# lukashermann/hulc

Hardware: AMD Instinct MI355X
Metric: trajectory-windows/sec (seq_len=32, bs=64/GPU) (higher is better)
Workload: dtype bf16; 1 GPU; HULC training step, vision goal only (use_clip_auxiliary_loss=false), B=64 windows/GPU, seq_len=32, 200x200 static + 84x84 gripper fp32 NCHW frames, fwd+loss+bwd+Adam, dropout 0.1; global_batch=64, seq_len=32, parallelism=dp1

## Files before the change

### hulc_amd/csrc/capi.hip

```cpp
#include <cstdarg>
#include <cstdio>
#include <cstring>
#include <cstdlib>
#include <cmath>
#include <algorithm>
#include <stdexcept>

#include "engine.h"
#include "sbert.h"
#include "store_gather.h"
#include "store_stage.h"

using namespace hulc_bf16;

static thread_local char g_err[1024] = "";
void hulc_set_error(const char* fmt, ...) {
    va_list ap;
    va_start(ap, fmt);
    vsnprintf(g_err, sizeof(g_err), fmt, ap);
    va_end(ap);
}

struct hulc_ctx {
    IEngine* e = nullptr;
// ... 316 lines not shown
    HULC_K_16BIT("hulc_k_enc_tail_bwd", k_enc_tail_bwd(Nf, ldemb, a, b, demb, stream));
}
int hulc_k_tr_layer_fwd(int32_t dtype, const hulc_tr_layer_job* job, int32_t B, int32_t S, int32_t ln_in, float dp, void* stream) {
    HULC_K_16BIT("hulc_k_tr_layer_fwd", k_tr_layer_fwd(job, B, S, ln_in, dp, stream));
}
int hulc_k_tr_ffn_bwd(int32_t dtype, const hulc_tr_ffn_bwd_job* job, int32_t B, int32_t S, int32_t bcast, float bdiv, float dp, void* stream) {
    HULC_K_16BIT("hulc_k_tr_ffn_bwd", k_tr_ffn_bwd(job, B, S, bcast, bdiv, dp, stream));
}
int hulc_k_tr_attn_bwd(int32_t dtype, const hulc_tr_attn_bwd_job* job, int32_t B, int32_t S, int32_t nparts, int64_t part_stride, float dp, void* stream) {
    HULC_K_16BIT("hulc_k_tr_attn_bwd", k_tr_attn_bwd(job, B, S, nparts, (long long)part_stride, dp, stream));
}
int hulc_k_gemm_multi(int32_t dtype, int32_t form, const hulc_gemm_epi_job* jobs, int32_t n, int32_t sh, int32_t* ran, void* stream) {
    HULC_K_16BIT("hulc_k_gemm_multi", k_gemm_multi(form, jobs, n, sh, ran, stream));
}
#undef HULC_K_16BIT
int hulc_k_gemm_epi(int32_t dtype, const hulc_gemm_epi_job* job, int32_t kernel, int32_t* ran, void* stream) {
    if (dtype == HULC_DTYPE_F16) return hulc_f16::k_gemm_epi(1, job, kernel, ran, stream);
    if (dtype != HULC_DTYPE_F32 && dtype != HULC_DTYPE_BF16) { hulc_set_error("hulc_k_gemm_epi: unknown dtype %d", (int)dtype); return 1; }
    return hulc_bf16::k_gemm_epi(dtype == HULC_DTYPE_BF16 ? 1 : 0, job, kernel, ran, stream);
}
int hulc_k_gemm_pick(int32_t dtype, int32_t M, int32_t N, int32_t K, int64_t lda, int64_t ldb, int32_t* pick, int32_t* bk) {
    if (dtype != HULC_DTYPE_F32 && dtype != HULC_DTYPE_BF16 && dtype != HULC_DTYPE_F16) { hulc_set_error("hulc_k_gemm_pick: unknown dtype %d", (int)dtype); return 1; }
    return hulc_bf16::k_gemm_pick(dtype != HULC_DTYPE_F32, M, N, K, (long long)lda, (long long)ldb, pick, bk);
}
int hulc_k_gemm_wgrad_nsplit(int32_t dtype, int32_t M, int32_t N, int32_t K, int32_t* nsplit, int32_t* big) {
    if (dtype != HULC_DTYPE_F32 && dtype != HULC_DTYPE_BF16 && dtype != HULC_DTYPE_F16) { hulc_set_error("hulc_k_gemm_wgrad_nsplit: unknown dtype %d", (int)dtype); return 1; }
    return hulc_bf16::k_gemm_wgrad_nsplit(dtype != HULC_DTYPE_F32, M, N, K, nsplit, big);
}
int hulc_k_logistic_loss(int32_t dtype, int32_t wide, const float* heads, int32_t ldh, const float* actions, const float* robot_obs, int32_t B, int32_t S,
                         int32_t n_mix, int32_t n_dim, int32_t num_classes, float log_scale_min, float gripper_alpha, int32_t gripper_control,
                         int32_t discrete_gripper, float grad_scale, const float* lscale, float* row_loss, float* a_tcp_out, void* dheads, void* stream) {
    if (dtype == HULC_DTYPE_F16)
        return hulc_f16::k_logistic_loss(1, wide, heads, ldh, actions, robot_obs, B, S, n_mix, n_dim, num_classes, log_scale_min, gripper_alpha, gripper_control,
                                         discrete_gripper, grad_scale, lscale, row_loss, a_tcp_out, dheads, stream);
    if (dtype != HULC_DTYPE_F32 && dtype != HULC_DTYPE_BF16) { hulc_set_error("hulc_k_logistic_loss: unknown dtype %d", (int)dtype); return 1; }
    return hulc_bf16::k_logistic_loss(dtype == HULC_DTYPE_BF16, wide, heads, ldh, actions, robot_obs, B, S, n_mix, n_dim, num_classes, log_scale_min, gripper_alpha,
                                      gripper_control, discrete_gripper, grad_scale, lscale, row_loss, a_tcp_out, dheads, stream);
}
#define HULC_K_ANY(name, fn, ...)                                                                                                     \
    if (dtype == HULC_DTYPE_F16) return hulc_f16::fn(1, __VA_ARGS__);                                                                  \
    if (dtype != HULC_DTYPE_F32 && dtype != HULC_DTYPE_BF16) { hulc_set_error(name ": unknown dtype %d", (int)dtype); return 1; }      \
    return hulc_bf16::fn(dtype == HULC_DTYPE_BF16 ? 1 : 0, __VA_ARGS__)
int hulc_k_plan_kl_sample(const float* pr_logits, const float* pp_logits, int32_t B, int32_t NCAT, int32_t NCLS, const int32_t* idx_in, int32_t* idx_out, float* probs,
                          float* kl_cat, float* dpp, float* dpr, float w_pp, float w_pr, uint64_t seed, const float* lscale, void* stream) {
    return hulc_bf16::k_plan_kl_sample(pr_logits, pp_logits, B, NCAT, NCLS, idx_in, idx_out, probs, kl_cat, dpp, dpr, w_pp, w_pr, (unsigned long long)seed, lscale, stream);
}
int hulc_k_st_softmax_bwd(int32_t dtype, const float* probs, const float* dplan, const float* dpr_kl, const float* dpp_kl, int32_t rows, int32_t NCLS, float* out, void* out_t,
                          void* dpp_t, void* stream) {
    HULC_K_ANY("hulc_k_st_softmax_bwd", k_st_softmax_bwd, probs, dplan, dpr_kl, dpp_kl, rows, NCLS, out, out_t, dpp_t, stream);
}
int hulc_k_plan_gather(int32_t dtype, const void* w_t, const int32_t* idx, int32_t B, int32_t NCAT, int32_t NCLS, int32_t H, const float* b1, const float* b2, float* out,
                       const void* emb, void* embg, int32_t S, int32_t W, const void* goal, int32_t G, int32_t grow0, void* cb, void* stream) {
    HULC_K_ANY("hulc_k_plan_gather", k_plan_gather, w_t, idx, B, NCAT, NCLS, H, b1, b2, out, emb, embg, S, W, goal, G, grow0, cb, stream);
}
int hulc_k_plan_scatter_grad(int32_t dtype, int32_t form, const void* dC, const int32_t* idx, int32_t B, int32_t NCAT, int32_t NCLS, int32_t H, int32_t KIN, float* dw,
                             int32_t store, void* stream) {
    HULC_K_ANY("hulc_k_plan_scatter_grad", k_plan_scatter_grad, form, dC, idx, B, NCAT, NCLS, H, KIN, dw, store, stream);
}
int hulc_k_normal_kl_sample(int32_t dtype, const float* pr_state, const float* pp_state, int32_t B, int32_t n, const float* eps_in, float* eps_out, float* plan_f, void* plan_t,
                            float* kl_elem, float* dpp, float* dpr, float w_pp, float w_pr, uint64_t seed, const float* lscale, void* stream) {
    HULC_K_ANY("hulc_k_normal_kl_sample", k_normal_kl_sample, pr_state, pp_state, B, n, eps_in, eps_out, plan_f, plan_t, kl_elem, dpp, dpr, w_pp, w_pr, (unsigned long long)seed, lscale, stream);
}
int hulc_k_normal_rsample_bwd(int32_t dtype, const float* dplan, const float* eps, const float* pr_state, const float* dpr_kl, int32_t B, int32_t n, void* out, void* stream) {
    HULC_K_ANY("hulc_k_normal_rsample_bwd", k_normal_rsample_bwd, dplan, eps, pr_state, dpr_kl, B, n, out, stream);
}
int hulc_k_det_head_loss(int32_t dtype, const void* H1, const void* W, const float* bias, const float* actions, const float* robot_obs, int32_t B, int32_t S,
                         int32_t criterion, int32_t frame, float grad_scale, const float* lscale, float* row_loss, float* pred, float* dpre, void* stream) {
    HULC_K_ANY("hulc_k_det_head_loss", k_det_head_loss, H1, W, bias, actions, robot_obs, B, S, criterion, frame, grad_scale, lscale, row_loss, pred, dpre, stream);
}
int hulc_k_det_head_bwd(int32_t dtype, const float* dpre, const void* W, const void* H1, int32_t B, int32_t S, void* dH1, void* dZ1, float* dW, float* db, void* stream) {
    HULC_K_ANY("hulc_k_det_head_bwd", k_det_head_bwd, dpre, W, H1, B, S, dH1, dZ1, dW, db, stream);
}
int hulc_k_det_head_act(int32_t dtype, const void* h1, const void* W, const float* bias, const float* robot_obs, int32_t n, float* out, void* stream) {
    HULC_K_ANY("hulc_k_det_head_act", k_det_head_act, h1, W, bias, robot_obs, n, out, stream);
}
int hulc_k_layernorm_fwd(int32_t dtype, const float* x, int64_t ldx, int32_t rows, int32_t n, const float* g, const float* b, void* out, int64_t ldo, float* out_f32, int64_t ldf,
                         float* stats, void* stream) {
    HULC_K_ANY("hulc_k_layernorm_fwd", k_layernorm_fwd, x, (long long)ldx, rows, n, g, b, out, (long long)ldo, out_f32, (long long)ldf, stats, stream);
}
int hulc_k_layernorm_bwd(int32_t dtype, const float* dy, int64_t lddy, const float* x, int64_t ldx, const float* stats, const float* g, int32_t rows, int32_t n, float* dx_f32,
                         int64_t ldd, int32_t accumulate, void* dx_t, int64_t ldt, float* dg, float* db, float drop_p, uint64_t seed, int32_t bcast_rows, float bcast_div,
                         int32_t dy_parts, int64_t dy_part_stride, float* scratch, void* stream) {
    HULC_K_ANY("hulc_k_layernorm_bwd", k_layernorm_bwd, dy, (long long)lddy, x, (long long)ldx, stats, g, rows, n, dx_f32, (long long)ldd, accumulate, dx_t, (long long)ldt, dg, db,
               drop_p, (unsigned long long)seed, bcast_rows, bcast_div, dy_parts, (long long)dy_part_stride, scratch, stream);
}
int hulc_k_layernorm_mean(int32_t dtype, const float* x, int32_t B, int32_t S, int32_t n, const float* g, const float* b, float* stats, void* out, float* yout, void* stream) {
    HULC_K_ANY("hulc_k_layernorm_mean", k_layernorm_mean, x, B, S, n, g, b, stats, out, yout, stream);
}
#undef HULC_K_ANY
int hulc_k_cast(int32_t dtype, const float* src, void* dst, int64_t n, void* stream) {
    hipStream_t st = (hipStream_t)stream;
    if (dtype == HULC_DTYPE_F32) hipLaunchKernelGGL((cast_kernel<float, float>), dim3(1024), dim3(256), 0, st, src, (float*)dst, (long long)n);
    else hipLaunchKernelGGL((cast_kernel<float, h16_t>), dim3(1024), dim3(256), 0, st, src, (h16_t*)dst, (long long)n);
    if (hipGetLastError() != hipSuccess) { hulc_set_error("hulc_k_cast: launch failed"); return 1; }
    return 0;
}
int hulc_k_window_compact(const int64_t* window_start, const int32_t* lens, const int32_t* off, int32_t off_base, int32_t B, int32_t S, int64_t store_frames,
                          const int32_t* shift_static, const int32_t* shift_gripper, int64_t* frame_out, int32_t* shift_static_out, int32_t* shift_gripper_out, void* stream) {
    if (!window_start || !lens || !off || !frame_out || B < 1 || S < 1 || store_frames < 1 || (shift_static && !shift_static_out) || (shift_gripper && !shift_gripper_out)) {
        hulc_set_error("hulc_k_window_compact: null argument or B=%d, S=%d, store_frames=%lld out of range", (int)B, (int)S, (long long)store_frames); return 1; }
    launch_window_compact((hipStream_t)stream, reinterpret_cast<const long long*>(window_start), lens, off, off_base, B, S, (long long)store_frames, shift_static, shift_gripper,
                          reinterpret_cast<long long*>(frame_out), shift_static_out, shift_gripper_out);
    if (hipGetLastError() != hipSuccess) { hulc_set_error("hulc_k_window_compact: launch failed"); return 1; }
    return 0;
}
int hulc_k_rows_expand(int32_t elem_bytes, const void* src, const int32_t* lens, const int32_t* off, int32_t B, int32_t S, int32_t n, void* dst, void* stream) {
// ... 201 lines not shown
```

### hulc_amd/csrc/engine.h

```cpp
#pragma once
#include <algorithm>
#include <map>
#include <string>
#include <vector>

#include "iengine.h"
#include "gemm.h"
#include "kernels.h"
#include "plan_ln_launch.h"
#include "conv_wgrad.h"
#include "conv_tile.h"
#include "conv_reg.h"
#include "tr_fused.h"
#include "rnn_persist.h"
#include "enc_tail.h"
#include "rollout_step.h"
#include "aux_heads.h"
#include "aux_rows.h"
#include "det_head.h"

namespace HULC_NS {

#define HIP_CHECK_VOID(x) do { hipError_t e_ = (x); if (e_ != hipSuccess) { hulc_set_error("%s:%d %s", __FILE__, __LINE__, hipGetErrorString(e_)); } } while (0)

// ... 11 lines not shown
    struct Ref { int64_t off, n; };
    std::map<std::string, Ref> tab;
    std::vector<void*> allocs;
    int64_t ws_bytes = 0;
    struct Named { void* p; int64_t n; int kind; };
    std::map<std::string, Named> named;

    template <typename U> U* alloc(int64_t n, const char* name = nullptr, int kind = -1) {
        void* p = nullptr;
        int64_t bytes = ((n * (int64_t)sizeof(U) + 255) / 256) * 256 + 256;
        if (hipMalloc(&p, bytes) != hipSuccess) { alloc_failed = true; return nullptr; }
        hipMemsetAsync(p, 0, bytes, st);
        allocs.push_back(p);
        ws_bytes += bytes; alloc_sz[p] = bytes;
        if (name) named[name] = Named{p, n, kind >= 0 ? kind : (std::is_same<U, float>::value ? 0 : (std::is_same<U, int>::value ? 2 : 1))};
        return (U*)p;
    }
    bool alloc_failed = false;
    std::map<void*, int64_t> alloc_sz;

    struct LinW {
        const float* W32 = nullptr; const float* b32 = nullptr; float* dW = nullptr; float* db = nullptr;
        T* W = nullptr; T* Wt = nullptr; int N = 0, K = 0; bool own_w = false;
        T* Wfr = nullptr; T* Wtfr = nullptr;
    };
    struct ConvW {
        const float* W32 = nullptr; const float* b32 = nullptr; float* dW = nullptr; float* db = nullptr;
        T* Wf = nullptr; T* Wd = nullptr; int O = 0, I = 0, KH = 0, KW = 0, S = 0; int nhwc = 0;
    };
    struct EncW { ConvW c1, c2, c3; LinW fc7, fc1, fc2; const float *lng = nullptr, *lnb = nullptr; float *dlng = nullptr, *dlnb = nullptr; bool gripper = false; int IH = 0; int H1 = 0, H2 = 0, H3 = 0; };
    EncW encS, encG;
    LinW pp[5], vg[3], lg[3], tr_in[2], tr_out[2], tr_l1[2], tr_l2[2], pr_fc, pr_fs, whh0, wih1, whh1, cl_im0, cl_im2, cl_la0, cl_la2;
    LinW bw_ih[2][2], bw_hh[2][2];
    const float *bb_ih[2][2], *bb_hh[2][2]; float *dbb_ih[2][2], *dbb_hh[2][2];
    T* gcarB2 = nullptr;
    T *bZ0[2] = {nullptr, nullptr}, *bH0[2], *bZ1, *bH1, *bh1b, *bxcat, *bdx, *bdH0[2], *bdZ0[2], *bdZ1, *bdz1b, *plan_t;
    float *plan_f, *plan_eps, *plan_eps_in, *klel;
    struct GruBuf { T *Zx, *H, *R, *Z, *N, *GN, *dZx, *dG; } gb[4];
    float* gGf = nullptr; T *gcarA = nullptr, *gcarB = nullptr;
    const float *ln_vg_g, *ln_vg_b, *ln_lg_g, *ln_lg_b, *tr_n1g[2], *tr_n1b[2], *tr_n2g[2], *tr_n2b[2], *pos32, *logit_scale;
    float *d_ln_vg_g, *d_ln_vg_b, *d_ln_lg_g, *d_ln_lg_b, *d_tr_n1g[2], *d_tr_n1b[2], *d_tr_n2g[2], *d_tr_n2b[2], *dpos, *dlogit_scale;
    const float *wih0_32, *bih0, *bhh0, *bih1, *bhh1;
    float *dwih0, *dbih0, *dbhh0, *dbih1, *dbhh1;
    T *wih0 = nullptr, *wih0T = nullptr;
    T *wheads = nullptr, *wheadsT = nullptr; float* bheads = nullptr; float *dwheads_tmp = nullptr, *dbheads_tmp = nullptr;
    const float *head_w32[4], *head_b32[4]; float *head_dw[4], *head_db[4]; int head_rows[4] = {60, 60, 60, 2};
    float* dw7_tmp = nullptr;
    bool bound = false;
    T* wshadow = nullptr;
    std::vector<TrDesc> trdesc; TrDesc* trdesc_dev = nullptr; int tr_blocks = 0; unsigned short* blk2desc_dev = nullptr;
    struct TrTable { TrDesc* desc = nullptr; unsigned short* b2d = nullptr; int blocks = 0, n = 0; };
    TrTable tr_adam, tr_rest;
    long long* adam_chunk_start = nullptr; int* adam_chunk_n = nullptr; int adam_chunks = 0;
    bool adam_fuse_tr = true;
    void set_adam_fuse(bool on) override { adam_fuse_tr = on; }
    bool frag_by_adam = false;
    bool rest_by_pack = false;
    bool tr_fresh = false;
    void tr_table_free(TrTable& t) { if (t.desc) hipFree(t.desc); if (t.b2d) hipFree(t.b2d); t = TrTable{}; }
    bool tr_table_build(TrTable& t, std::vector<TrDesc> v) {
        tr_table_free(t);
        int blk = 0;
        for (TrDesc& d : v) { d.blk0 = blk; blk += d.tiles_x * cdiv(d.R, TRT); }
        t.blocks = blk; t.n = (int)v.size();
        if (v.empty()) return true;
        std::vector<unsigned short> b2d((size_t)blk);
        for (size_t i = 0; i < v.size(); ++i) { const int end = i + 1 < v.size() ? v[i + 1].blk0 : blk; for (int b = v[i].blk0; b < end; ++b) b2d[b] = (unsigned short)i; }
        if (hipMalloc((void**)&t.desc, sizeof(TrDesc) * v.size()) != hipSuccess || hipMalloc((void**)&t.b2d, sizeof(unsigned short) * b2d.size()) != hipSuccess) return false;
        hipMemcpy(t.desc, v.data(), sizeof(TrDesc) * v.size(), hipMemcpyHostToDevice);
        hipMemcpy(t.b2d, b2d.data(), sizeof(unsigned short) * b2d.size(), hipMemcpyHostToDevice);
        return true;
    }
    void adam_tables_build() {
        tr_table_free(tr_adam); tr_table_free(tr_rest); rest_by_pack = false; frag_by_adam = false;
        if (adam_chunk_start) { hipFree(adam_chunk_start); adam_chunk_start = nullptr; } if (adam_chunk_n) { hipFree(adam_chunk_n); adam_chunk_n = nullptr; }
        adam_chunks = 0;
        if (std::is_same<T, float>::value || !wshadow || (numel & 3)) return;
        std::vector<TrDesc> fused, rest;
        std::vector<std::pair<long long, long long>> rng;
        for (const TrDesc& d : trdesc) {
            const T* src = (const T*)d.src;
            const long long off = src - wshadow;
            const bool in = src >= wshadow && off + (long long)d.R * d.C <= numel && d.lds == d.C && (d.C & 3) == 0 && (off & 3) == 0 && !d.cs;
            if (in) { fused.push_back(d); rng.emplace_back(off, off + (long long)d.R * d.C); } else rest.push_back(d);
        }
        std::sort(rng.begin(), rng.end());
        for (size_t i = 0; i + 1 < rng.size(); ++i) if (rng[i].second > rng[i + 1].first) return;
        if (fused.empty() || fused.size() > 65535) return;
        std::vector<long long> cs; std::vector<int> cn;
        long long pos = 0;
        auto cover = [&](long long lo, long long hi) { for (long long x = lo; x < hi; x += ADAM_CHUNK) { cs.push_back(x); cn.push_back((int)std::min<long long>(ADAM_CHUNK, hi - x)); } };
        for (auto& r : rng) { cover(pos, r.first); pos = r.second; }
        cover(pos, numel);
        if (!tr_table_build(tr_adam, fused) || !tr_table_build(tr_rest, rest)) { tr_table_free(tr_adam); tr_table_free(tr_rest); return; }
        { int lf = 0; for (const TrDesc& d : fused) if (d.fr && d.frT) ++lf; frag_by_adam = fragbatch.n > 0 && 2 * lf == fragbatch.n && lf == frag_linked; }
        rest_by_pack = true;
        for (const TrDesc& d : rest) {
            const bool f7 = d.src == (const void*)encG.fc7.W && d.dst == (void*)encG.fc7.Wt && d.R == 128 && d.C == 3136 && d.ldt == 128;
            const bool hd = d.src == (const void*)wheads && d.dst == (void*)wheadsT && d.R == NHEAD && d.C == HID && d.ldt == NHEAD;
            if (!f7 && !hd) rest_by_pack = false;
        }
        adam_chunks = (int)cs.size();
        if (adam_chunks) {
            if (hipMalloc((void**)&adam_chunk_start, sizeof(long long) * cs.size()) != hipSuccess || hipMalloc((void**)&adam_chunk_n, sizeof(int) * cn.size()) != hipSuccess) { tr_table_free(tr_adam); tr_table_free(tr_rest); adam_chunks = 0; return; }
            hipMemcpy(adam_chunk_start, cs.data(), sizeof(long long) * cs.size(), hipMemcpyHostToDevice);
            hipMemcpy(adam_chunk_n, cn.data(), sizeof(int) * cn.size(), hipMemcpyHostToDevice);
        }
    }

    struct EncA {
        T *a1, *a2, *a3, *ss, *g0, *f1; float *ssstats, *f2, *lnst; unsigned* m1bits = nullptr; unsigned* m2bits = nullptr;
        T *dact1 = nullptr, *dact2 = nullptr, *dact3 = nullptr, *d_f1 = nullptr, *d_f2t = nullptr, *d_g0 = nullptr; float* d_ss = nullptr;
    } aS, aG;
    T *emb, *lang_t, *gl1, *gl2, *goal_t, *ppx, *ppa[4], *xm, *seqf_t, *embg, *Cb, *Zx0, *Zx1, *H0, *H1, *dheads, *dH1, *dZ1, *dH0, *dZ0, *dC;
    float *gl3, *goal_st, *pp_logits, *seqf, *pr_logits, *probs, *klcat, *dpp_kl, *dpr_kl, *Cplan, *heads, *rowloss, *a_tcp;
    int* pidx; int* pidx_in;
    T *xt[3], *qkv[2], *ao[2], *x1t[2], *hff[2];
    float *xf[3], *Pat[2], *y1[2], *st1[2], *x1f[2], *y2[2], *st2[2];
    float* zero_arena = nullptr; int64_t zero_n = 0; bool arena_clean = false;
    int* work_ctrs = nullptr; int work_ctr_next = 0;
    int* next_ctr() { return work_ctrs ? work_ctrs + (work_ctr_next++ & 63) : nullptr; }
    float *demb, *dgoal, *dseqf, *dplan, *dprl, *dppx, *dxa, *dxb, *dy_f, *dxm;
    T *dprl_t, *dppl_t, *dseq_t, *dt_a, *dt_b, *dt_c, *dgl3_t;
    T *tA, *tB; int64_t tcap;
    bool h0t_valid = false;
    T* tB2 = nullptr;
    float *part; int64_t partcap; float* cspart;
    int* auxrows; T *sf_m, *im1, *g_m, *la1, *img_t, *txt_t; float *img, *txt, *dimg, *dtxt, *dsf_m, *dg_m; T *dimg_t, *dtxt_t, *dim1, *dla1;
    float* losses;
    bool aux_bcz = false, aux_mia = false;
    float aux_w_bcz = 1.f, aux_w_mia = 1.f;
    LinW bz0, bz2;
    const float *mia_w0 = nullptr, *mia_b0 = nullptr, *mia_w1 = nullptr, *mia_b1 = nullptr;
    float *d_mia_w0 = nullptr, *d_mia_b0 = nullptr, *d_mia_w1 = nullptr, *d_mia_b1 = nullptr;
    T *bz1 = nullptr, *dbz1 = nullptr, *bz_dpred_t = nullptr; float *bz_pred = nullptr, *bz_tgt = nullptr, *bz_dpred = nullptr;
    float* aux_loss = nullptr;
    int bcz_n = 0, mia_n = 0;
    float *clip_rows_ws = nullptr, *mia_rows_ws = nullptr;
    int aux_rows_last = 0;
    bool det = false, dec_selected = false; int det_crit = HULC_CRIT_HUBER;
    const float *det_w32 = nullptr, *det_b32 = nullptr; float *det_dw = nullptr, *det_db = nullptr;
    const T* det_w = nullptr;
    float* dpre = nullptr;
    hulc_batch cur{}; float cur_lw = 0, cur_cw = 0; bool have_fwd = false;

    Engine(const hulc_config& c) : cfg(c) {
        memset(&cur2, 0, sizeof(cur2));
        mcil = cfg.kind == HULC_KIND_MCIL || cfg.kind == HULC_KIND_MCIL_GRU;
        gru = cfg.kind == HULC_KIND_MCIL_GRU;
        PLAN = mcil ? 512 : 1024; NDIM = mcil ? 7 : 6; NO = NMIX * NDIM; NHEAD = mcil ? 224 : 192; DE = mcil ? EMB : 64;
        if (mcil) { head_rows[0] = head_rows[1] = head_rows[2] = NO; head_rows[3] = 0; }
        dec_plan = cfg.kind == HULC_KIND_GCBC ? 0 : (mcil ? PLAN / 2 : PLAN);
        KIN = dec_plan + DE + GOAL;
        maxB = cfg.max_batch; maxS = cfg.max_seq; maxN = maxB * maxS;
    }
    ~Engine() override { for (void* p : allocs) hipFree(p); if (rp_err_host) hipHostFree((void*)rp_err_host); if (blk2desc_dev) hipFree(blk2desc_dev); if (trdesc_dev) hipFree(trdesc_dev); tr_table_free(tr_adam); tr_table_free(tr_rest); if (adam_chunk_start) hipFree(adam_chunk_start); if (adam_chunk_n) hipFree(adam_chunk_n); gn_free(); if (clip_state) hipFree(clip_state); if (env_rows_host) hipHostFree(env_rows_host); }
    int64_t workspace_bytes() const override { return ws_bytes; }
    void set_kl_beta(float b) override { cfg.kl_beta = b; }
    void set_dropout(float p) override { cfg.dropout_p = p; }

    uint64_t site_seed(int site) const {
        uint64_t z = cfg.seed + 0x9E3779B97F4A7C15ull * (cur.step * 64 + (cur.is_lang ? 32 : 0) + site + 1);
        z = (z ^ (z >> 30)) * 0xBF58476D1CE4E5B9ull; z = (z ^ (z >> 27)) * 0x94D049BB133111EBull; return z ^ (z >> 31);
    }

    void alloc_enc(EncA& a, int IH, bool gripper, const char* pre) {
        const int H1 = (IH - 8) / 4 + 1, H2 = (H1 - 4) / 2 + 1, H3 = H2 - 2;
        std::string s(pre);
        a.a1 = alloc<T>((int64_t)maxN * H1 * H1 * 32, (s + "a1").c_str());
        a.m1bits = std::is_same<T, h16_t>::value ? alloc<unsigned>((int64_t)maxN * H1 * H1) : nullptr;
        a.a2 = alloc<T>((int64_t)maxN * H2 * H2 * 64, (s + "a2").c_str());
        a.m2bits = std::is_same<T, h16_t>::value ? alloc<unsigned>((int64_t)maxN * H2 * H2 * 2) : nullptr;
        a.a3 = alloc<T>((int64_t)maxN * H3 * H3 * 64, (s + "a3").c_str());
        a.ss = gripper ? nullptr : alloc<T>((int64_t)maxN * 128, (s + "ss").c_str());
        a.ssstats = gripper ? nullptr : alloc<float>((int64_t)maxN * 64 * 4);
        a.g0 = gripper ? alloc<T>((int64_t)maxN * 128, (s + "g0").c_str()) : nullptr;
        a.f1 = alloc<T>((int64_t)maxN * 512, (s + "f1").c_str());
        a.f2 = alloc<float>((int64_t)maxN * 64, (s + "f2").c_str());
        a.lnst = alloc<float>((int64_t)maxN * 2);
    }
    int alloc_all() {
        const int64_t N = maxN, B = maxB, S = maxS, SB = (int64_t)maxS * maxB;
        alloc_enc(aS, 200, false, "s_");
        alloc_enc(aG, 84, true, "g_");
        aS.dact1 = alloc<T>(N * 49 * 49 * 32, "dact1"); aS.dact2 = alloc<T>(N * 23 * 23 * 64, "dact2"); aS.dact3 = alloc<T>(N * 21 * 21 * 64, "dact3");
        aG.d_g0 = alloc<T>(N * 128); aS.d_f1 = alloc<T>(N * 512); aS.d_f2t = alloc<T>(N * 64); aS.d_ss = alloc<float>(N * 128, "d_ss");
        if constexpr (std::is_same<T, h16_t>::value) {
            aG.d_f1 = alloc<T>(N * 512); aG.d_f2t = alloc<T>(N * 64);
            aG.dact1 = alloc<T>(N * 20 * 20 * 32, "g_dact1"); aG.dact2 = alloc<T>(N * 9 * 9 * 64, "g_dact2"); aG.dact3 = alloc<T>(N * 7 * 7 * 64, "g_dact3");
        } else {
            aG.d_f1 = aS.d_f1; aG.d_f2t = aS.d_f2t; aG.dact1 = aS.dact1; aG.dact2 = aS.dact2; aG.dact3 = aS.dact3;
        }
        emb = alloc<T>(N * EMB, "emb"); lang_t = alloc<T>(B * LANG); gl1 = alloc<T>(B * HID); gl2 = alloc<T>(B * HID);
        gl3 = alloc<float>(B * GOAL, "goal_pre"); goal_t = alloc<T>(B * GOAL, "goal"); goal_st = alloc<float>(B * 2);
        ppx = alloc<T>(B * (EMB + GOAL)); for (int i = 0; i < 4; ++i) ppa[i] = alloc<T>(B * HID);
        pp_logits = alloc<float>(B * PLAN, "pp_logits");
        for (int l = 0; l < 3; ++l) { xt[l] = alloc<T>(N * EMB); xf[l] = alloc<float>(N * EMB, l == 2 ? "pr_x_final" : (l == 0 ? "pr_x0" : "pr_x1")); }
        for (int l = 0; l < 2; ++l) {
            qkv[l] = alloc<T>(N * 3 * EMB); Pat[l] = alloc<float>(B * NH * S * S, l ? "attn_p1" : "attn_p0"); ao[l] = alloc<T>(N * EMB);
            y1[l] = alloc<float>(N * EMB); st1[l] = alloc<float>(N * 2); x1t[l] = alloc<T>(N * EMB); x1f[l] = alloc<float>(N * EMB);
            hff[l] = alloc<T>(N * FF); y2[l] = alloc<float>(N * EMB); st2[l] = alloc<float>(N * 2);
        }
        xm = alloc<T>(B * EMB); seqf = alloc<float>(B * FCH, "seq_feat"); seqf_t = alloc<T>(B * FCH); pr_logits = alloc<float>(B * PLAN, "pr_logits");
        probs = alloc<float>(B * PLAN, "pr_probs"); klcat = alloc<float>(B * NCAT); dpp_kl = alloc<float>(B * PLAN); dpr_kl = alloc<float>(B * PLAN);
        pidx = alloc<int>(B * NCAT, "plan_idx"); pidx_in = alloc<int>(B * NCAT);
        embg = alloc<T>(SB * DE); Cplan = alloc<float>(B * HID); Cb = alloc<T>(B * HID, "dec_cb");
        Zx0 = alloc<T>(SB * HID); Zx1 = alloc<T>(SB * HID); H0 = alloc<T>(SB * HID, "dec_h0"); H1 = alloc<T>(SB * HID, "dec_h1");
        heads = alloc<float>(SB * NHEAD, "heads"); dheads = alloc<T>(SB * NHEAD, "dheads"); rowloss = alloc<float>(SB * 8); a_tcp = alloc<float>(SB * 7, "a_tcp");
        dH1 = alloc<T>(SB * HID); dZ1 = alloc<T>(SB * HID, "dec_dz1"); dH0 = alloc<T>(SB * HID); dZ0 = alloc<T>(SB * HID, "dec_dz0"); dC = alloc<T>(B * HID);
// ... 407 lines not shown
    void gemm_wgrad(const DenseLoader<T>& a, const DenseLoader<T>& b, float* dW, long long lddw, int M, int N, int K) {
        EpiP ep = epi(dW, true); ep.accumulate = 1;
        if constexpr (std::is_same<T, h16_t>::value) {
            if (a.R1 == 0x7fffffff && b.R1 == 0x7fffffff && skinny_ok(M, N, K, a.s1, b.s1, a.p, b.p)) { gemm(a, b, dense_out(lddw), ep, M, N, K); return; }
        }
        bool big = false;
        const int nsplit = gemm_wgrad_nsplit<T>(M, N, K, &big);
        if (nsplit <= 1) { gemm(a, b, dense_out(lddw), ep, M, N, K); return; }
        ep.atomic = 1;
        TimerScope ts(this, big ? "gemm_128x128" : "gemm_64x64_splitk", "mfma", 2.0 * M * N * K, ((double)M * K + (double)N * K) * sizeof(T) + 4.0 * M * N);
        if (big) launch_gemm<T, 128, 128>(st, a, b, dense_out(lddw), ep, M, N, K, 1, nsplit);
        else launch_gemm<T, 64, 64>(st, a, b, dense_out(lddw), ep, M, N, K, 1, nsplit);
    }
    EpiP epi(void* out, bool f32) const { EpiP e; e.out = out; e.out_f32 = f32 ? 1 : 0; e.generic_only = epilogue_fast ? 0 : 1; return e; }

    void lin_fwd(const T* X, long long ldx, int M, const LinW& L, EpiP ep, long long ldo) {
        if (!ep.bias) ep.bias = L.b32;
        gemm(dense<T>(X, M, ldx), dense<T>(L.W, L.N, L.K), dense_out(ldo), ep, M, L.N, L.K);
    }
    void lin_wgrad(const T* dY, const T* X, long long ldx, int M, int N, int K, float* dW, long long lddw, float* db, float* db2 = nullptr) {
        if constexpr (std::is_same<T, h16_t>::value) {
            if (M <= 64) {
                hipLaunchKernelGGL(lin_bwd_smallm_kernel, dim3(cdiv(N, 64), cdiv(K, 128)), dim3(256), 0, st, dY, (long long)N, X, ldx, M, N, K, dW, lddw, db, db2, 64, grad_first(dW) ? 1 : 0);
                return;
            }
            grad_ensure_zero(dW);
        }
        const int mp = ldpad(M);
        constexpr bool fuse_cs = std::is_same<T, h16_t>::value;
        transpose_pair(dY, N, tA, M, N, X, ldx, tB, M, K, mp, fuse_cs ? db : nullptr, fuse_cs ? db2 : nullptr);
        gemm_wgrad(dense<T>(tA, N, mp), dense<T>(tB, K, mp), dW, lddw, N, K, M);
        if (db && !fuse_cs) colsum(dY, N, M, N, db, db2);
    }
    void lin_dgrad(const T* dY, int M, const LinW& L, EpiP ep, const DenseOut& om) {
        gemm(dense<T>(dY, M, L.N), dense<T>(L.Wt, L.K, L.N), om, ep, M, L.K, L.N);
    }
    void ln_fwd(const float* x, long long ldx, int rows, int n, const float* g, const float* b, T* out, long long ldo, float* outf, long long ldf,
                float* stats) {
        launch_ln_fwd<T>(st, x, ldx, rows, n, g, b, out, ldo, outf, ldf, stats);
    }
    static constexpr bool ln_bwd_can_bcast = ln_bwd_fused<T>();
    void ln_bwd(const float* dy, long long lddy, const float* x, long long ldx, const float* stats, const float* g, int rows, int n, float* dxf,
                long long ldd, int acc, T* dxt, long long ldt, float* dg, float* db, float drop_p = 0.f, unsigned long long drop_seed = 0,
                int bcast_rows = 0, float bcast_div = 1.f, int dy_parts = 1, long long dy_part_stride = 0) {
        launch_ln_bwd<T>(st, cspart, dy, lddy, x, ldx, stats, g, rows, n, dxf, ldd, acc, dxt, ldt, dg, db, drop_p, drop_seed, bcast_rows, bcast_div, dy_parts, dy_part_stride);
    }

    int prepare_weights(bool shadow_fresh = false) override {
        if (!bound) { hulc_set_error("hulc_prepare_weights before hulc_bind_params"); return 1; }
        c1_bias_fold_valid = false;
        if constexpr (!std::is_same<T, float>::value) {
            if (!shadow_fresh) hipLaunchKernelGGL((cast_kernel<float, T>), dim3(2048), dim3(256), 0, st, P, wshadow, (long long)numel);
        }
        {
            ConvPackBatch d;
            int k = 0, blk = 0;
            for (EncW* e : {&encS, &encG})
                for (ConvW* c : {&e->c1, &e->c2, &e->c3}) {
                    d.w[k] = c->W32; d.wf[k] = c->Wf; d.wd[k] = c->nhwc ? c->Wd : nullptr; d.O[k] = c->O; d.I[k] = c->I; d.K[k] = c->KH; d.S[k] = c->S; d.nhwc[k] = c->nhwc;
                    d.blk0[k] = blk; blk += cdiv(c->O * c->I * c->KH * c->KW, 256); ++k;
                }
            d.blk0[6] = blk;
            const int blkA = blk, blkB = blkA + cdiv(128 * 3136, 256);
            const HeadPack hp = head_pack();
            const int rows = head_rows[0] + head_rows[1] + head_rows[2] + head_rows[3];
            T* const f7t = rest_by_pack ? encG.fc7.Wt : (T*)nullptr;
            T* const wht = rest_by_pack ? wheadsT : (T*)nullptr;
            hipLaunchKernelGGL((weight_pack_kernel<T>), dim3(blkB + cdiv((long long)rows * HID, 256)), dim3(256), 0, st, d, blkA, encG.fc7.W32, encG.fc7.W, 128, 64, 49, blkB, hp,
                               wheads, bheads, HID, f7t, wht, NHEAD);
        }
        if (std::is_same<T, float>::value) hipLaunchKernelGGL((batched_transpose_kernel<float, T>), dim3(tr_blocks), dim3(256), 0, st, trdesc_dev, (int)trdesc.size());
        else if (tr_fresh && tr_adam.n) {
            if (tr_rest.blocks && !rest_by_pack) hipLaunchKernelGGL(batched_transpose64_kernel, dim3(tr_rest.blocks), dim3(256), 0, st, tr_rest.desc, tr_rest.n, (const unsigned short*)tr_rest.b2d);
        }
        else hipLaunchKernelGGL(batched_transpose64_kernel, dim3(tr_blocks), dim3(256), 0, st, trdesc_dev, (int)trdesc.size(), (const unsigned short*)blk2desc_dev);
        const bool was_fresh = tr_fresh && tr_adam.n;
        tr_fresh = false;
        if constexpr (std::is_same<T, h16_t>::value) {
            if (fragbatch.n && !(was_fresh && frag_by_adam)) hipLaunchKernelGGL(frag_pack_kernel, dim3(frag_blocks), dim3(256), 0, st, fragbatch);
        }
        if (hipGetLastError() != hipSuccess) { hulc_set_error("kernel launch failed in prepare_weights"); return 1; }
        return 0;
    }
    T *trb_c[2] = {nullptr, nullptr}, *trb_a[2] = {nullptr, nullptr}, *trb_d[2] = {nullptr, nullptr}, *trb_b[2] = {nullptr, nullptr};
    LinBwdBatch tr_wjobs{};
    int tr_wblocks = 0;
    void tr_wgrad_add(const T* dY, const T* X, const LinW& L) {
        if constexpr (std::is_same<T, h16_t>::value) {
            LinBwdJob& J = tr_wjobs.j[tr_wjobs.n++];
            J.dY = dY; J.X = X; J.dW = L.dW; J.db = L.db; J.ldx = L.K; J.lddw = L.K; J.N = L.N; J.K = L.K; J.nx = cdiv(L.N, 64); J.blk0 = tr_wblocks; J.part = nullptr;
            tr_wblocks += J.nx * cdiv(L.K, 128);
        }
    }
    void tr_wgrads_flush(int M) {
        if constexpr (std::is_same<T, h16_t>::value) {
            if (tr_wjobs.n == 0) return;
            const int chunk = 256, nz = cdiv(M, chunk);
            tr_wjobs.M = M; tr_wjobs.store = 0; tr_wjobs.mchunk = chunk;
            UnpackBatch ub{};
            int64_t cur = 0; int ublocks = 0;
            for (int i = 0; i < tr_wjobs.n; ++i) {
                LinBwdJob& J = tr_wjobs.j[i];
                const int64_t need = (int64_t)nz * J.N * J.K;
                if (part_cur + cur + need > this->partcap) { J.part = nullptr; continue; }
                J.part = this->part + part_cur + cur; cur += need;
                UnpackJob& U = ub.j[ub.n++];
                U.part = J.part; U.grad = J.dW; U.slab = (long long)J.N * J.K; U.nsplit = nz; U.O = J.N; U.I = J.K; U.KH = U.KW = 1; U.nhwc = 0; U.blk0 = ublocks; U.ysplit = 1;
// ... 138 lines not shown
        const ClipState h{total, coef, clip_algo, clip_limit};
        HIP_CHECK(hipMemcpyAsync(clip_state, &h, sizeof(h), hipMemcpyHostToDevice, st));
        HIP_CHECK(hipStreamSynchronize(st));
        return 0;
    }
    int grad_clip_set(int32_t algo, float limit, int32_t track) override {
        if (algo != HULC_CLIP_OFF && algo != HULC_CLIP_NORM && algo != HULC_CLIP_VALUE) { hulc_set_error("hulc_grad_clip_set: unknown algorithm %d", (int)algo); return 1; }
        if (!(limit > 0.f)) algo = HULC_CLIP_OFF;
        if ((algo == HULC_CLIP_NORM || track != 0) && bound && !gn_built && gn_build()) return 1;
        clip_algo = algo; clip_limit = algo == HULC_CLIP_OFF ? 0.f : limit; clip_track = track != 0;
        gn_have = false;
        if (clip_algo == HULC_CLIP_OFF && !clip_track) return 0;
        return clip_state_write(0.f, 1.f);
    }
    int grad_norm_get(float* total, float* coef, float* per_tensor, int64_t cap) override {
        if (!gn_have) { hulc_set_error("hulc_grad_norm_get: no optimizer step has computed gradient norms (hulc_grad_clip_set with HULC_CLIP_NORM or track != 0 first)"); return 1; }
        if (per_tensor && cap < (int64_t)gn_tens.size()) { hulc_set_error("hulc_grad_norm_get: per-tensor buffer holds %lld values, %lld tensors are bound", (long long)cap, (long long)gn_tens.size()); return 1; }
        ClipState h;
        HIP_CHECK(hipMemcpyAsync(&h, clip_state, sizeof(h), hipMemcpyDeviceToHost, st));
        if (per_tensor) HIP_CHECK(hipMemcpyAsync(per_tensor, gn_tnorm, sizeof(float) * gn_tens.size(), hipMemcpyDeviceToHost, st));
        HIP_CHECK(hipStreamSynchronize(st));
        if (total) *total = h.total_norm;
        if (coef) *coef = h.coef;
        return 0;
    }

    int optim(const hulc_optim& o) override {
        if (!bound) { hulc_set_error("hulc_optimizer_step before hulc_bind_params"); return 1; }
        const bool want_norm = clip_algo == HULC_CLIP_NORM || clip_track;
        if (want_norm && !gn_built) { hulc_set_error("hulc_optimizer_step: the gradient-norm tables are missing (hulc_bind_params / hulc_grad_clip_set build them)"); return 1; }
        persist_check("hulc_optimizer_step", false);
        lazy_sweep(0, numel, st);
        bwd_since_opt = false;
        const unsigned tag = ++opt_seq;
        if (o.kind != HULC_OPT_ADAM && o.kind != HULC_OPT_ADAMW && o.kind != HULC_OPT_SGD) { hulc_set_error("hulc_optimizer_step: unknown optimizer kind %d", (int)o.kind); return 1; }
        if (o.step < 1) { hulc_set_error("hulc_optimizer_step: step counts from 1 (got %lld)", (long long)o.step); return 1; }
        const float lr = o.lr, b1 = o.beta1, b2 = o.beta2, eps = o.eps, gscale = o.grad_scale;
        const int64_t step = o.step;
        const double bc1d = 1.0 - pow((double)b1, (double)step), bc2d = 1.0 - pow((double)b2, (double)step);
        h16_t* const shadow = std::is_same<T, float>::value ? (h16_t*)nullptr : (h16_t*)wshadow;
        const ClipState* const cs = clip_algo != HULC_CLIP_OFF ? clip_state : nullptr;
        if (want_norm) {
            hipLaunchKernelGGL(grad_sumsq_kernel, dim3(gn_chunks), dim3(256), 0, st, (const float*)G, (const long long*)gn_chunk_start, (const int*)gn_chunk_n, gn_partial, scaler);
            hipLaunchKernelGGL(grad_norm_combine_kernel, dim3(1), dim3(1024), 0, st, (const float*)gn_partial, (const int*)gn_tfirst, (int)gn_tens.size(), gscale, (const ScalerState*)scaler,
                               clip_state, gn_tsq, gn_tnorm);
            gn_have = true;
        } else if (scaler) hipLaunchKernelGGL(nonfinite_check_kernel, dim3(2048), dim3(256), 0, st, G, (long long)numel, scaler);
        if (o.kind == HULC_OPT_SGD)
            hipLaunchKernelGGL(sgd_kernel, dim3(2048), dim3(256), 0, st, P, G, AM, (long long)numel, lr, o.momentum, o.dampening, o.weight_decay, (int)(o.nesterov != 0),
                               (int)(step == 1), gscale, shadow, (const ScalerState*)scaler, (const unsigned*)rp_skip, tag, cs);
        else if (adam_fuse_tr && tr_adam.n && shadow) {
            AdamArgs a{P, G, AM, AV, lr, b1, b2, eps, (float)bc1d, (float)sqrt(bc2d), gscale, o.weight_decay, (int)(o.kind == HULC_OPT_ADAMW), shadow, (const ScalerState*)scaler, (const unsigned*)rp_skip, tag, cs};
            hipLaunchKernelGGL(adam_tiled_kernel, dim3(tr_adam.blocks + adam_chunks), dim3(256), 0, st, a, (const TrDesc*)tr_adam.desc, (const unsigned short*)tr_adam.b2d, tr_adam.blocks,
                               (const long long*)adam_chunk_start, (const int*)adam_chunk_n);
            tr_fresh = true;
        } else
            hipLaunchKernelGGL(adam_kernel, dim3(2048), dim3(256), 0, st, P, G, AM, AV, (long long)numel, lr, b1, b2, eps, (float)bc1d, (float)sqrt(bc2d), gscale,
                               shadow, (const ScalerState*)scaler, o.weight_decay, (int)(o.kind == HULC_OPT_ADAMW), (const unsigned*)rp_skip, tag, cs);
        if (scaler) hipLaunchKernelGGL(scaler_update_kernel, dim3(1), dim3(1), 0, st, scaler, (const unsigned*)rp_skip, tag);
        if (hipGetLastError() != hipSuccess) { hulc_set_error("adam launch failed"); return 1; }
        return prepare_weights(true);
    }

    int get_tensor(const char* name, float* out, int64_t cap, int64_t* n) override {
        auto it = named.find(name);
        if (it == named.end()) { hulc_set_error("hulc_get_tensor: unknown tensor '%s'", name); return 1; }
        const Named& t = it->second;
        int64_t cnt = std::min<int64_t>(cap, t.n);
        *n = cnt;
        HIP_CHECK(hipStreamSynchronize(st));
        if (t.kind == 0) { HIP_CHECK(hipMemcpy(out, t.p, cnt * sizeof(float), hipMemcpyDeviceToHost)); }
        else if (t.kind == 1) {
            std::vector<T> tmp(cnt);
            HIP_CHECK(hipMemcpy(tmp.data(), t.p, cnt * sizeof(T), hipMemcpyDeviceToHost));
            for (int64_t i = 0; i < cnt; ++i) out[i] = host_to_f(tmp[i]);
        } else {
            std::vector<int> tmp(cnt);
            HIP_CHECK(hipMemcpy(tmp.data(), t.p, cnt * sizeof(int), hipMemcpyDeviceToHost));
            for (int64_t i = 0; i < cnt; ++i) out[i] = (float)tmp[i];
        }
        return 0;
    }
    static float host_to_f(float x) { return x; }
#ifdef HULC_HALF_F16
    static float host_to_f(h16_t x) {
        const uint32_t sgn = (uint32_t)(x >> 15) << 31, ex = (x >> 10) & 31, man = x & 1023;
        uint32_t u;
        if (ex == 0) { float f = ldexpf((float)man, -24); memcpy(&u, &f, 4); u |= sgn; }
        else if (ex == 31) u = sgn | 0x7f800000u | (man << 13);
        else u = sgn | ((ex + 112) << 23) | (man << 13);
        float f; memcpy(&f, &u, 4); return f;
    }
#else
    static float host_to_f(h16_t x) { uint32_t u = ((uint32_t)x) << 16; float f; memcpy(&f, &u, 4); return f; }
#endif
    int get_plan_idx(int32_t* out, int64_t cap) override {
        HIP_CHECK(hipStreamSynchronize(st));
        int64_t cnt = std::min<int64_t>(cap, (int64_t)cur.B * NCAT);
        HIP_CHECK(hipMemcpy(out, pidx, cnt * sizeof(int), hipMemcpyDeviceToHost));
        return 0;
    }
};

int k_gemm_nt(int is_f32, const void* A, const void* B, float* C, int M, int N, int K, long long lda, long long ldb, long long ldc, const float* bias, int relu,
              void* stream) {
    hipStream_t st = (hipStream_t)stream;
    EpiP ep; ep.out = C; ep.out_f32 = 1; ep.bias = bias; ep.relu = relu & 1;
    if (!is_f32 && !(relu & 4) && M >= 512 && N >= 128) {
// ... 35 lines not shown
```

### hulc_amd/csrc/engine_backward.inc

```
    struct Bucket { int64_t lo, hi; };
    Bucket group_range(const char* prefix) const {
        int64_t lo = numel, hi = 0;
        const std::string a(prefix);
        for (size_t i = 0; i < tab_order.size(); ++i) {
            const auto& kv = tab_order[i];
            if (kv.first.compare(0, a.size(), a) == 0) { lo = std::min(lo, kv.second.off); hi = std::max(hi, i + 1 < tab_order.size() ? tab_order[i + 1].second.off : numel); }
        }
        if (hi <= lo) return Bucket{0, 0};
        return Bucket{lo, std::min<int64_t>(hi, numel)};
    }
    std::vector<std::pair<std::string, Ref>> tab_order;
    std::vector<Bucket> bucket_plan() const {
        std::vector<Bucket> v;
        const Bucket dec = group_range("action_decoder.");
        v.push_back(Bucket{dec.lo, numel});
        v.push_back(group_range("plan_proposal."));
        v.push_back(group_range("plan_recognition."));
        const Bucket vg = group_range("visual_goal."), lg = group_range("language_goal.");
        v.push_back(Bucket{std::min(vg.lo, lg.lo), std::max(vg.hi, lg.hi)});
        v.push_back(group_range("perceptual_encoder."));
        return v;
    }
    int comm_buckets(int64_t* lo, int64_t* hi, int cap) override {
        if (!bound) { hulc_set_error("hulc_comm_buckets before hulc_bind_params"); return -1; }
// ... 353 lines not shown
                    }
                } else {
                    if (S <= 32) hipLaunchKernelGGL((attention_bwd_kernel<T, 32>), dim3(B * NH), dim3(64), 0, st, qkv[l], Pat[l], dt_a, B, S, EMB, NH, b_b, dp, site_seed(1 + 4 * l));
                    else hipLaunchKernelGGL((attention_bwd_kernel<T, 64>), dim3(B * NH), dim3(64), 0, st, qkv[l], Pat[l], dt_a, B, S, EMB, NH, b_b, dp, site_seed(1 + 4 * l));
                }
                if (defer_w) tr_wgrad_add(b_b, xt[l], tr_in[l]);
                else lin_wgrad(b_b, xt[l], EMB, N, 3 * EMB, EMB, tr_in[l].dW, EMB, tr_in[l].db);
                { EpiP ep = epi(dx, true); ep.res = dy_f; ep.res_f32 = 1; ep.res_ld = EMB; lin_dgrad(b_b, N, tr_in[l], ep, dense_out(EMB)); }
            }
            tr_wgrads_flush(N);
            {
                const int bchunk = std::is_same<T, float>::value ? B : 8;
                hipLaunchKernelGGL(pr_input_bwd_kernel, dim3(cdiv(S * EMB, 256), cdiv(B, bchunk)), dim3(256), 0, st, dx, B, S, EMB, dp, site_seed(0), demb, dpos, bchunk);
            }
        }
        if (bucket_ready(1) || bucket_ready(2)) return 1;
        if (pair) {
            const int Bv = pairBv, Bl = B - pairBv;
            T* av[2] = {gl1, gl2};
            T* al[2] = {gl1 + (long long)Bv * HID, gl2 + (long long)Bv * HID};
            ln_bwd(dgoal, GOAL, gl3, GOAL, goal_st, ln_vg_g, Bv, GOAL, nullptr, 0, 0, dgl3_t, GOAL, d_ln_vg_g, d_ln_vg_b);
            DenseOut om = dense_out((long long)S * EMB);
            mlp_bwd(dgl3_t, emb + (long long)(S - 1) * EMB, (long long)S * EMB, Bv, vg, 3, av, dt_a, dt_a + (long long)B * HID, demb + (long long)(S - 1) * EMB, &om, 1);
            ln_bwd(dgoal + Bv * GOAL, GOAL, gl3 + Bv * GOAL, GOAL, goal_st + 2 * Bv, ln_lg_g, Bl, GOAL, nullptr, 0, 0, dgl3_t + Bv * GOAL, GOAL, d_ln_lg_g, d_ln_lg_b);
            mlp_bwd(dgl3_t + Bv * GOAL, lang_t, LANG, Bl, lg, 3, al, dt_a, dt_a + (long long)B * HID, nullptr, nullptr, 0);
        } else {
            T* acts[2] = {gl1, gl2};
            if (b->is_lang) {
                ln_bwd(dgoal, GOAL, gl3, GOAL, goal_st, ln_lg_g, B, GOAL, nullptr, 0, 0, dgl3_t, GOAL, d_ln_lg_g, d_ln_lg_b);
                mlp_bwd(dgl3_t, lang_t, LANG, B, lg, 3, acts, dt_a, dt_a + (long long)B * HID, nullptr, nullptr, 0);
            } else {
                ln_bwd(dgoal, GOAL, gl3, GOAL, goal_st, ln_vg_g, B, GOAL, nullptr, 0, 0, dgl3_t, GOAL, d_ln_vg_g, d_ln_vg_b);
                DenseOut om = dense_out((long long)S * EMB);
                mlp_bwd(dgl3_t, emb + (long long)(S - 1) * EMB, (long long)S * EMB, B, vg, 3, acts, dt_a, dt_a + (long long)B * HID,
                        demb + (long long)(S - 1) * EMB, &om, 1);
            }
        }
        }
        if (bucket_ready(3)) return 1;
        if (part == 0) {
            lazy_sweep(0, numel, st);
            if (hipGetLastError() != hipSuccess) { hulc_set_error("kernel launch failed in backward"); return 1; }
            bwd_stage = 1;
            return 0;
        }
    encoders:
        {
            const Conv1Src src[2] = {conv1_src(*b, false), conv1_src(*b, true)}, src2[2] = {conv1_src(cur2, false), conv1_src(cur2, true)};
            const bool tail_fused = enc_tail_fusable();
            const int Nenc = enc_frames(N);
            if (ragged()) launch_rows_reduce(st, demb, rg_lens(), rg_off(), B, S, EMB, demb_c);
            if (tail_fused) enc_tail_bwd_both(Nenc);
            enc_bwd_both(src, pair ? src2 : nullptr, Nenc, tail_fused);
            flush_unpacks();
        }
        if (bucket_ready(4)) return 1;
        lazy_sweep(0, numel, st);
        if (hipGetLastError() != hipSuccess) { hulc_set_error("kernel launch failed in backward"); return 1; }
        have_fwd = false;
        bwd_stage = 0;
        grads_fresh = false;
        return 0;
    }
```

### hulc_amd/csrc/engine_encoders.inc

```
    ConvGeom geom(int Nf, int IH, int C, int K, int S) const {
        ConvGeom g; g.Nf = Nf; g.IH = g.IW = IH; g.C = C; g.KH = g.KW = K; g.S = S; g.OH = g.OW = (IH - K) / S + 1; return g;
    }
    Conv1Src conv1_src(const hulc_batch& b, bool gripper) const {
        Conv1Src s;
        s.X = gripper ? b.rgb_gripper : b.rgb_static;
        s.u8 = b.frames_u8 != 0;
        s.shift = s.u8 ? (gripper ? b.shift_gripper : b.shift_static) : nullptr;
        s.pad = gripper ? b.pad_gripper : b.pad_static;
        s.fold = (s.u8 && std::is_same<T, h16_t>::value && u8_fold_mode) ? 1 : 0;
        if (s.u8 && b.window_start) { s.wstart = reinterpret_cast<const long long*>(b.window_start); s.S = b.S; s.nstore = b.store_frames; }
        if (s.wstart && (b.window_len || b.window_len_host)) {
            const int set = &b == &cur2 ? 1 : 0;
            s.wstart = wl_frame[set]; s.S = 1;
            if (s.shift) s.shift = wl_shift[set][gripper ? 1 : 0];
        }
        return s;
    }
    static Conv1Src conv1_src_f32(const void* x) { return Conv1Src{x, nullptr, 0, 0}; }
    long long* wl_frame[2] = {nullptr, nullptr};
    int* wl_shift[2][2] = {{nullptr, nullptr}, {nullptr, nullptr}};
    int wl_alloc(int set) {
        if (!wl_frame[set]) {
            wl_frame[set] = alloc<long long>((int64_t)maxN); wl_shift[set][0] = alloc<int>((int64_t)maxN * 2); wl_shift[set][1] = alloc<int>((int64_t)maxN * 2);
            if (alloc_failed) { hulc_set_error("window_len: workspace allocation failed"); return 1; }
// ... 158 lines not shown
            const Stage S = stage(0, sn, Nf), G = stage(1, sn, Nf);
            const ConvTileP j[2] = {conv_fwd_job(S), conv_fwd_job(G)};
            TimerScope ts(this, "conv_tile_fwd", "mfma", 0, 0, 0);
            const bool ok = sn == 2 ? launch_conv_reg_fwd_jobs<32, 4, 4, 2>(st, j, 2) : launch_conv_reg_fwd_jobs<64, 3, 3, 1>(st, j, 2);
            if (ok) ts.add(conv_fwd_flops(S.c, S.g) + conv_fwd_flops(G.c, G.g), conv_fwd_bytes(S.c, S.g) + conv_fwd_bytes(G.c, G.g));
            return ok;
        }
        return false;
    }
    void enc_fwd_stages(int k0, int k1, const Conv1Src* src, const Conv1Src* src2, int Nf, bool defer_tail) {
        const bool both = k1 - k0 == 2;
        for (int k = k0; k < k1; ++k) conv1_fwd(k, src[k], Nf, src2 ? &src2[k] : nullptr);
        for (int sn = 2; sn <= 3; ++sn)
            if (!(both && conv_fwd_both(sn, Nf))) for (int k = k0; k < k1; ++k) conv_fwd(k, sn, Nf);
        for (int k = k0; k < k1; ++k) head_fwd(k, Nf, defer_tail);
    }
    void enc_fwd_both(const Conv1Src* src, const Conv1Src* src2, int Nf, bool defer_tail) {
        if constexpr (std::is_same<T, h16_t>::value) enc_fwd_stages(0, 2, src, src2, Nf, defer_tail);
        else for (int k = 0; k < 2; ++k) enc_fwd_stages(k, k + 1, src, src2, Nf, defer_tail);
    }
    bool enc_tail_fusable() const {
        if constexpr (!std::is_same<T, h16_t>::value) return false;
        auto ok = [](const EncW& e) { return e.fc1.K == 128 && e.fc1.N == 512 && e.fc2.K == 512 && e.fc2.N == 64; };
        return ok(encS) && ok(encG) && EMB == 128;
    }
    bool x0_done = false;
    void enc_tail_fwd_both(int Nf, bool with_x0 = false, int S = 1, float dp = 0.f) {
        if constexpr (std::is_same<T, h16_t>::value) {
            EncTailP q{};
            if (with_x0) { q.pos = pos32; q.xf = xf[0]; q.xt = xt[0]; q.z0 = y2[0]; q.z1 = y2[1]; q.S = S; q.drop_p = dp; q.seed = site_seed(0); x0_done = true; }
            for (int k = 0; k < 2; ++k) {
                const EncW& e = encw(k); EncA& a = enca(k);
                EncTailCam& c = q.cam[k];
                c.x = e.gripper ? a.g0 : a.ss; c.W1 = e.fc1.W; c.W2 = e.fc2.W; c.b1 = e.fc1.b32; c.b2 = e.fc2.b32;
                c.lng = e.lng; c.lnb = e.lnb; c.f1 = a.f1; c.f2 = a.f2; c.lnst = a.lnst; c.col0 = k * 64;
            }
            q.emb = enc_emb(); q.Nf = Nf; q.ldemb = EMB;
            launch_enc_tail_fwd(st, q);
        }
    }
    UnpackBatch unpack_jobs{};
    int64_t part_cur = 0;
    int unpack_blocks = 0;
    bool unpack_room(int jobs, int64_t floats) const { return unpack_jobs.n + jobs <= UNPACK_MAX_JOBS && part_cur + floats <= this->partcap; }
    float* queue_unpack(float* grad, int O, int I, int KH, int KW, int nhwc, int nsplit, int ysplit) {
        const long long slab = (long long)O * I * KH * KW;
        if (!unpack_room(1, nsplit * slab)) return nullptr;
        float* const slabs = this->part + part_cur;
        UnpackJob& U = unpack_jobs.j[unpack_jobs.n++];
        U.part = slabs; U.grad = grad; U.slab = slab; U.nsplit = nsplit; U.O = O; U.I = I; U.KH = KH; U.KW = KW; U.nhwc = nhwc; U.blk0 = unpack_blocks; U.ysplit = ysplit;
        unpack_blocks += cdiv((int)slab, 1024); part_cur += nsplit * slab;
        return slabs;
    }
    void flush_unpacks() {
        constexpr int yparts = 8;
        if (unpack_jobs.n > 0) hipLaunchKernelGGL(unpack_conv_wgrad_batched_kernel, dim3(unpack_blocks, yparts), dim3(256), 0, st, unpack_jobs);
        unpack_jobs.n = 0; part_cur = 0; unpack_blocks = 0;
    }
    bool tail_fc7_done = false;
    void enc_tail_bwd_both(int Nf) {
        if constexpr (std::is_same<T, h16_t>::value) {
            EncTailBwdP q{};
            for (int k = 0; k < 2; ++k) {
                const EncW& e = encw(k); EncA& a = enca(k);
                EncTailBwdCam& c = q.cam[k];
                c.f2 = a.f2; c.lnst = a.lnst; c.lng = e.lng; c.f1 = a.f1; c.W2t = e.fc2.Wt; c.W1t = e.fc1.Wt;
                c.xmask = a.g0; c.dlng = e.dlng; c.dlnb = e.dlnb;
                c.d_f2 = a.d_f2t; c.d_f1 = a.d_f1; c.dx_f32 = a.d_ss; c.dx_t = a.d_g0; c.col0 = k * 64;
            }
            q.demb = enc_demb(); q.Nf = Nf; q.ldemb = EMB;
            launch_enc_tail_bwd(st, q);
            constexpr int chunk = 256;
            LinBwdBatch bt{}; bt.M = Nf; bt.store = 0; bt.mchunk = chunk;
            int blk = 0;
            const int nz = cdiv(Nf, chunk);
            auto add = [&](const T* dY, const T* X, const LinW& L, float* dW, float* slabs) {
                LinBwdJob& J = bt.j[bt.n++];
                J.dY = dY; J.X = X; J.dW = dW; J.db = L.db; J.ldx = L.K; J.lddw = L.K; J.N = L.N; J.K = L.K; J.nx = cdiv(L.N, 64); J.blk0 = blk; J.part = slabs;
                blk += J.nx * cdiv(L.K, 128);
            };
            for (int k = 0; k < 2; ++k) {
                const EncW& e = encw(k); EncA& a = enca(k);
                add(a.d_f2t, a.f1, e.fc2, e.fc2.dW, queue_unpack(e.fc2.dW, e.fc2.N, e.fc2.K, 1, 1, 0, nz, 1));
                add(a.d_f1, e.gripper ? a.g0 : a.ss, e.fc1, e.fc1.dW, queue_unpack(e.fc1.dW, e.fc1.N, e.fc1.K, 1, 1, 0, nz, 1));
            }
            const LinW& L = encG.fc7;
            float* const slabs7 = L.N == 128 && L.K == 3136 ? queue_unpack(L.dW, 128, 64, 7, 7, 1, nz, 1) : nullptr;
            tail_fc7_done = slabs7 != nullptr;
            if (slabs7) add(aG.d_g0, aG.a3, L, nullptr, slabs7);
            hipLaunchKernelGGL(lin_bwd_smallm_batched_kernel, dim3(blk, nz), dim3(256), 0, st, bt);
        }
    }
    h16_t* zero_page = nullptr;
    const h16_t* wgrad_zero_page() {
        if constexpr (std::is_same<T, h16_t>::value) { if (!zero_page) zero_page = alloc<h16_t>(128); }
        return zero_page;
    }
    template <int TM, typename LB> int wgrad_gemm(const ConvW& c, const T* dy, const LB& lb, long long npix) {
        const int Kc = c.I * c.KH * c.KW;
        int nsplit = (int)std::min<long long>(std::max<long long>(1, npix / 2048), (this->partcap - part_cur) / ((long long)c.O * Kc));
        nsplit = std::min(nsplit, 256);
        EpiP ep = epi(this->part + part_cur, true); ep.z_stride = (long long)c.O * Kc;
        PixMajorLoaderT<T> la{}; la.p = dy; la.rows = c.O; la.ld = c.O;
        launch_gemm<T, TM, 64>(st, la, lb, dense_out(Kc), ep, c.O, Kc, (int)npix, 1, nsplit);
        return nsplit;
    }
    void wgrad_unpack(const ConvW& c, const T* dy, long long npix, int nsplit, bool bias_done) {
        const bool many = std::is_same<T, h16_t>::value && nsplit >= 64;
        if (!(many && queue_unpack(c.dW, c.O, c.I, c.KH, c.KW, c.nhwc, nsplit, 0)))
// ... 215 lines not shown
```

### hulc_amd/csrc/iengine.h

```cpp
#pragma once
#include <hip/hip_runtime.h>
#include <cstring>
#include <map>
#include <string>
#include <vector>

#include "../../include/hulc_hip.h"
#include "comm.h"

void hulc_set_error(const char* fmt, ...);

struct IEngine {
    virtual ~IEngine() { delete comm; delete comm_pending; }
    virtual int bind(float* p, float* g, float* m, float* v, int64_t numel, int n, const char* const* names, const int64_t* offs,
                     const int64_t* numels) = 0;
    virtual int prepare_weights(bool shadow_fresh = false) = 0;
    virtual int zero_grads() = 0;
    virtual int flush_grads() = 0;
    virtual int forward(const hulc_batch* b, float lw, float cw, float* out, int on_host) = 0;
    virtual int forward_pair(const hulc_batch* vis, const hulc_batch* lang, float lw, float cw, float* out8, int on_host) = 0;
    virtual int backward(int part = -1) = 0;
    virtual int validate(const hulc_batch* b, const hulc_val_noise* nz, float* out17, int32_t* plan_pp_out, int32_t* plan_pr_out, float* pred_pp_out,
                         float* pred_pr_out) = 0;
    virtual int clip_gt_encode(const float* lang_emb, int m, int slot) = 0;
// ... 92 lines not shown
            if (!e->timing_filter.empty() && e->timing_filter.find(std::string(",") + name + ",") == std::string::npos) return;
            e->timer_depth++;
            t = &e->timers[name];
            if (t->name.empty()) { t->name = name; t->bound = bound; }
            if (t->used == t->ev.size()) { hipEvent_t a, b; hipEventCreateWithFlags(&a, e->event_flags); hipEventCreateWithFlags(&b, e->event_flags); t->ev.emplace_back(a, b); }
            t->flops += flops; t->bytes += bytes; t->launches += nlaunch;
            hipEventRecord(t->ev[t->used].first, e->st);
        }
        void add(double flops, double bytes, int nlaunch = 1) { if (t) { t->flops += flops; t->bytes += bytes; t->launches += nlaunch; } }
        ~TimerScope() { if (t) { hipEventRecord(t->ev[t->used].second, e->st); t->used++; e->timer_depth--; } }
    };
    int timers_read(char* out, int64_t cap, bool reset) {
        hipStreamSynchronize(st);
        std::string js = "{";
        bool first = true;
        for (auto& kv : timers) {
            KTimer& t = kv.second;
            double ms = 0;
            for (size_t i = 0; i < t.used; ++i) { float x = 0; hipEventElapsedTime(&x, t.ev[i].first, t.ev[i].second); ms += x; }
            char buf[512];
            snprintf(buf, sizeof(buf), "%s\"%s\": {\"bound\": \"%s\", \"launches\": %lld, \"ms\": %.6f, \"flops\": %.6e, \"bytes\": %.6e}", first ? "" : ", ",
                     t.name.c_str(), t.bound.c_str(), t.launches, ms, t.flops, t.bytes);
            js += buf; first = false;
            if (reset) { t.used = 0; t.flops = t.bytes = 0; t.launches = 0; }
        }
        js += "}";
        if ((int64_t)js.size() + 1 > cap) { hulc_set_error("hulc_timers_read: buffer too small"); return 1; }
        memcpy(out, js.c_str(), js.size() + 1);
        return 0;
    }
};

#define HULC_TU_DECLS                                                                                                                         \
    IEngine* make_engine(const hulc_config& cfg, int* rc);                                                                                   \
    int k_gemm_nt(int is_f32, const void* A, const void* B, float* C, int M, int N, int K, long long lda, long long ldb, long long ldc, \
                  const float* bias, int relu, void* stream);                                                                                \
    int k_spatial_softmax64(const void* f, int H, int W, int Nf, void* out, float* stats, const float* dout, void* df, void* stream);          \
    int k_enc_tail_fwd(int Nf, int ldemb, const hulc_enc_tail_job* a, const hulc_enc_tail_job* b, void* emb, const float* pos, int S,           \
                       float drop_p, unsigned long long seed, float* xf, void* xt, float* z0, float* z1, void* stream);                         \
    int k_enc_tail_bwd(int Nf, int ldemb, const hulc_enc_tail_bwd_job* a, const hulc_enc_tail_bwd_job* b, const float* demb, void* stream);     \
    int k_logistic_loss(int t16, int wide, const float* heads, int ldh, const float* actions, const float* robot_obs, int B, int S, int nmix,   \
                        int ndim, int num_classes, float log_scale_min, float gripper_alpha, int gripper_control, int discrete_gripper,         \
                        float grad_scale, const float* lscale, float* row_loss, float* a_tcp_out, void* dheads, void* stream);                  \
    int k_det_head_loss(int t16, const void* H1, const void* W, const float* bias, const float* actions, const float* robot_obs, int B, int S, int criterion,     \
                        int frame, float grad_scale, const float* lscale, float* row_loss, float* pred, float* dpre, void* stream);                              \
    int k_det_head_bwd(int t16, const float* dpre, const void* W, const void* H1, int B, int S, void* dH1, void* dZ1, float* dW, float* db, void* stream);        \
    int k_det_head_act(int t16, const void* h1, const void* W, const float* bias, const float* robot_obs, int n, float* out, void* stream);                       \
    int k_plan_kl_sample(const float* pr_logits, const float* pp_logits, int B, int NCAT, int NCLS, const int* idx_in, int* idx_out, float* probs,  \
                         float* kl_cat, float* dpp, float* dpr, float w_pp, float w_pr, unsigned long long seed, const float* lscale, void* stream); \
    int k_st_softmax_bwd(int t16, const float* probs, const float* dplan, const float* dpr_kl, const float* dpp_kl, int rows, int NCLS, float* out,  \
                         void* out_t, void* dpp_t, void* stream);                                                                               \
    int k_plan_gather(int t16, const void* w_t, const int* idx, int B, int NCAT, int NCLS, int H, const float* b1, const float* b2, float* out,   \
                      const void* emb, void* embg, int S, int W, const void* goal, int G, int grow0, void* cb, void* stream);                     \
    int k_plan_scatter_grad(int t16, int form, const void* dC, const int* idx, int B, int NCAT, int NCLS, int H, int KIN, float* dw, int store,   \
                            void* stream);                                                                                                      \
    int k_normal_kl_sample(int t16, const float* pr_state, const float* pp_state, int B, int n, const float* eps_in, float* eps_out, float* plan_f, \
                           void* plan_t, float* kl_elem, float* dpp, float* dpr, float w_pp, float w_pr, unsigned long long seed,                 \
                           const float* lscale, void* stream);                                                                                  \
    int k_normal_rsample_bwd(int t16, const float* dplan, const float* eps, const float* pr_state, const float* dpr_kl, int B, int n, void* out,  \
                             void* stream);                                                                                                     \
    int k_layernorm_fwd(int t16, const float* x, long long ldx, int rows, int n, const float* g, const float* b, void* out, long long ldo,        \
                        float* out_f32, long long ldf, float* stats, void* stream);                                                             \
    int k_layernorm_bwd(int t16, const float* dy, long long lddy, const float* x, long long ldx, const float* stats, const float* g, int rows,    \
                        int n, float* dx_f32, long long ldd, int accumulate, void* dx_t, long long ldt, float* dg, float* db, float drop_p,       \
                        unsigned long long seed, int bcast_rows, float bcast_div, int dy_parts, long long dy_part_stride, float* scratch,        \
                        void* stream);                                                                                                          \
    int k_layernorm_mean(int t16, const float* x, int B, int S, int n, const float* g, const float* b, float* stats, void* out, float* yout,      \
                         void* stream);                                                                                                         \
    int k_tr_layer_fwd(const hulc_tr_layer_job* j, int B, int S, int ln_in, float dp, void* stream);                                            \
    int k_tr_ffn_bwd(const hulc_tr_ffn_bwd_job* j, int B, int S, int bcast, float bdiv, float dp, void* stream);                                \
    int k_tr_attn_bwd(const hulc_tr_attn_bwd_job* j, int B, int S, int nparts, long long part_stride, float dp, void* stream);                  \
    int k_gemm_epi(int t16, const hulc_gemm_epi_job* j, int kernel, int* ran, void* stream);                                                    \
    int k_gemm_multi(int form, const hulc_gemm_epi_job* jobs, int n, int sh, int* ran, void* stream);                                           \
    int k_gemm_pick(int t16, int M, int N, int K, long long lda, long long ldb, int* pick, int* bk);                                            \
    int k_gemm_wgrad_nsplit(int t16, int M, int N, int K, int* nsplit, int* big);                                                               \
    int k_conv_wgrad(const char* who, int typed, int which, const void* X, const void* dY, float* out, float* db_out, int Nf, int IH, int* slabs, \
                     void* stream);                                                                                                             \
    int k_conv1_wgrad_u8(const char* who, int typed, const void* X, const int* shifts, int pad, const void* dY, float* dw_out, float* db_out,   \
                         int Nf, int IH, int form, int fold, int* slabs, void* stream);                                                         \
    int k_conv_tile(const char* who, int typed, int mode, const void* img, const void* w, const float* bias, const void* mask, void* out,       \
                    unsigned* bits1_out, int Nf, int IMH, int OUTH, int relu, int wgs, void* stream);                                           \
    int k_conv_pair(const char* who, int typed, int stage, const hulc_conv_job* a, const hulc_conv_job* b, int wg_a, int wg_b, int* slabs,      \
                    void* stream);                                                                                                              \
    int k_conv_plan(int form, int frames, int in_side, int out_side, int wgs, int* nbands, int* rows_per_band, int* frames_per_band, int* items);
namespace hulc_bf16 { HULC_TU_DECLS }
namespace hulc_f16 { HULC_TU_DECLS }
```

### hulc_amd/csrc/k_entries.h

```cpp
#pragma once
#include "iengine.h"
#include "kernels.h"
#include "enc_tail.h"
#include "plan_ln_launch.h"
#include "gemm.h"
#include "tr_fused.h"
#include "det_head.h"
#include <vector>

namespace HULC_NS {

static inline bool k_misaligned16(const void* p) { return (reinterpret_cast<uintptr_t>(p) & 15) != 0; }
static inline int k_launched(const char* who) {
    const hipError_t e = hipGetLastError();
    if (e != hipSuccess) { hulc_set_error("%s: launch failed: %s", who, hipGetErrorString(e)); return 1; }
    return 0;
}

int k_spatial_softmax64(const void* f, int H, int W, int Nf, void* out, float* stats, const float* dout, void* df, void* stream) {
    hipStream_t st = (hipStream_t)stream;
    if (Nf < 1 || H < 2 || W < 2 || (long long)H * W > (1 << 20)) { hulc_set_error("hulc_k_spatial_softmax64: Nf=%d H=%d W=%d (need Nf >= 1, H, W >= 2)", Nf, H, W); return 1; }
    if (!f || !stats || (dout ? !df : !out)) { hulc_set_error("hulc_k_spatial_softmax64: null argument"); return 1; }
    if (k_misaligned16(f) || k_misaligned16(stats) || k_misaligned16(dout) || k_misaligned16(df)) { hulc_set_error("hulc_k_spatial_softmax64: f, stats, dout, df must be 16-byte aligned"); return 1; }
    if (!dout) hipLaunchKernelGGL(spatial_softmax_fwd64_kernel, dim3(Nf), dim3(256), 0, st, (const h16_t*)f, H, W, (h16_t*)out, stats);
// ... 149 lines not shown
    HULC_K_T("hulc_k_det_head_act", HULC_K_L);
#undef HULC_K_L
    return k_launched("hulc_k_det_head_act");
}

int k_plan_kl_sample(const float* pr_logits, const float* pp_logits, int B, int NCAT, int NCLS, const int* idx_in, int* idx_out, float* probs, float* kl_cat, float* dpp,
                     float* dpr, float w_pp, float w_pr, unsigned long long seed, const float* lscale, void* stream) {
    hipStream_t st = (hipStream_t)stream;
    if (B < 1 || NCAT < 1 || NCLS < 1 || NCLS > 64 || (long long)B * NCAT * NCLS > (1ll << 30)) { hulc_set_error("hulc_k_plan_kl_sample: B=%d NCAT=%d NCLS=%d (need B, NCAT >= 1 and 1 <= NCLS <= 64)", B, NCAT, NCLS); return 1; }
    if (!pr_logits || !idx_out || !probs || (pp_logits && (!kl_cat || !dpp || !dpr))) { hulc_set_error("hulc_k_plan_kl_sample: null argument"); return 1; }
    if (k_misaligned(pr_logits, 4) || k_misaligned(pp_logits, 4) || k_misaligned(idx_in, 4) || k_misaligned(idx_out, 4) || k_misaligned(probs, 4) || k_misaligned(kl_cat, 4) ||
        k_misaligned(dpp, 4) || k_misaligned(dpr, 4) || k_misaligned(lscale, 4)) { hulc_set_error("hulc_k_plan_kl_sample: every pointer must be 4-byte aligned"); return 1; }
    if (idx_in && k_idx_out_of_range("hulc_k_plan_kl_sample", idx_in, (long long)B * NCAT, NCLS, st)) return 1;
    hipLaunchKernelGGL(plan_kl_sample_kernel, dim3(B * NCAT), dim3(64), 0, st, pr_logits, pp_logits, B, NCAT, NCLS, idx_in, idx_out, probs, kl_cat, dpp, dpr, w_pp, w_pr, seed, lscale);
    return k_launched("hulc_k_plan_kl_sample");
}

int k_st_softmax_bwd(int t16, const float* probs, const float* dplan, const float* dpr_kl, const float* dpp_kl, int rows, int NCLS, float* out, void* out_t, void* dpp_t,
                     void* stream) {
    hipStream_t st = (hipStream_t)stream;
    if (rows < 1 || NCLS < 1 || NCLS > 64 || (long long)rows * NCLS > (1ll << 30)) { hulc_set_error("hulc_k_st_softmax_bwd: rows=%d NCLS=%d (need rows >= 1 and 1 <= NCLS <= 64)", rows, NCLS); return 1; }
    if (!probs || !dplan || !dpr_kl || !dpp_kl || !out || !out_t || !dpp_t) { hulc_set_error("hulc_k_st_softmax_bwd: null argument"); return 1; }
    const int ta = t16 ? 2 : 4;
    if (k_misaligned(probs, 4) || k_misaligned(dplan, 4) || k_misaligned(dpr_kl, 4) || k_misaligned(dpp_kl, 4) || k_misaligned(out, 4) || k_misaligned(out_t, ta) || k_misaligned(dpp_t, ta)) {
        hulc_set_error("hulc_k_st_softmax_bwd: a pointer is not aligned to its element type"); return 1;
    }
#define HULC_K_L(TT) hipLaunchKernelGGL((st_softmax_bwd_kernel<TT>), dim3(rows), dim3(64), 0, st, probs, dplan, dpr_kl, NCLS, out, (TT*)out_t, dpp_kl, (TT*)dpp_t)
    HULC_K_T("hulc_k_st_softmax_bwd", HULC_K_L);
#undef HULC_K_L
    return k_launched("hulc_k_st_softmax_bwd");
}

int k_plan_gather(int t16, const void* w_t, const int* idx, int B, int NCAT, int NCLS, int H, const float* b1, const float* b2, float* out, const void* emb, void* embg, int S,
                  int W, const void* goal, int G, int grow0, void* cb, void* stream) {
    hipStream_t st = (hipStream_t)stream;
    if (B < 1 || H < 256 || (H % 256) != 0 || NCAT < 0 || NCAT > 64 || NCLS < 1 || (long long)B * H > (1ll << 30)) {
        hulc_set_error("hulc_k_plan_gather: B=%d H=%d NCAT=%d NCLS=%d (need B >= 1, H a multiple of 256, 0 <= NCAT <= 64, NCLS >= 1)", B, H, NCAT, NCLS); return 1;
    }
    if (!w_t || !b1 || !b2 || !out || (NCAT > 0 && !idx) || (!emb != !embg) || (cb && !goal)) { hulc_set_error("hulc_k_plan_gather: null argument (emb and embg go together, cb needs goal)"); return 1; }
    if (embg && (S < 1 || W < 1 || W > 128 || (long long)S * B * W > (1ll << 30))) { hulc_set_error("hulc_k_plan_gather: embg given: S=%d W=%d (need S >= 1, 1 <= W <= 128)", S, W); return 1; }
    if (cb && (G < 1 || grow0 < NCAT * NCLS)) { hulc_set_error("hulc_k_plan_gather: cb given: G=%d grow0=%d (need G >= 1 and grow0 past the %d plan rows)", G, grow0, NCAT * NCLS); return 1; }
    const int ta = t16 ? 2 : 4;
    if (k_misaligned(w_t, ta) || k_misaligned(idx, 4) || k_misaligned(b1, 4) || k_misaligned(b2, 4) || k_misaligned(out, 4) || k_misaligned(emb, ta) || k_misaligned(embg, ta) ||
        k_misaligned(goal, ta) || k_misaligned(cb, ta)) { hulc_set_error("hulc_k_plan_gather: a pointer is not aligned to its element type"); return 1; }
    if (NCAT > 0 && k_idx_out_of_range("hulc_k_plan_gather", idx, (long long)B * NCAT, NCLS, st)) return 1;
    const int SBW = embg ? S * B * W : 0;
    if (!embg) { S = 0; W = 0; }
#define HULC_K_L(TT)                                                                                                                                             \
    hipLaunchKernelGGL((plan_gather_t_kernel<TT>), dim3(cdiv((long long)B * H, 256) + cdiv(SBW, 256)), dim3(256), 0, st, (const TT*)w_t, idx, B, NCAT, NCLS, H, b1, b2, out, \
                       (const TT*)emb, (TT*)embg, S, W, (const TT*)goal, G, grow0, (TT*)cb)
    HULC_K_T("hulc_k_plan_gather", HULC_K_L);
#undef HULC_K_L
    return k_launched("hulc_k_plan_gather");
}

int k_plan_scatter_grad(int t16, int form, const void* dC, const int* idx, int B, int NCAT, int NCLS, int H, int KIN, float* dw, int store, void* stream) {
    hipStream_t st = (hipStream_t)stream;
    if (B < 1 || NCAT < 1 || NCAT > 64 || NCLS < 1 || NCLS > 32 || H < 1 || KIN < NCAT * NCLS || (long long)B * H > (1ll << 30) || (long long)H * KIN > (1ll << 30)) {
        hulc_set_error("hulc_k_plan_scatter_grad: B=%d NCAT=%d NCLS=%d H=%d KIN=%d (need 1 <= NCAT <= 64, 1 <= NCLS <= 32: the LDS tile has 32 rows, KIN >= NCAT * NCLS)", B, NCAT, NCLS, H, KIN); return 1;
    }
    if (form != 0 && form != 1) { hulc_set_error("hulc_k_plan_scatter_grad: form must be 0 (lds) or 1 (w4), got %d", form); return 1; }
    if (store && form != 1) { hulc_set_error("hulc_k_plan_scatter_grad: store goes with form 1 (w4) only"); return 1; }
    if (store != 0 && store != 1) { hulc_set_error("hulc_k_plan_scatter_grad: store must be 0 or 1"); return 1; }
    if (!dC || !idx || !dw) { hulc_set_error("hulc_k_plan_scatter_grad: null argument"); return 1; }
    if (k_misaligned(dC, t16 ? 2 : 4) || k_misaligned(idx, 4) || k_misaligned(dw, 4)) { hulc_set_error("hulc_k_plan_scatter_grad: a pointer is not aligned to its element type"); return 1; }
    if (form == 1 && !(t16 ? plan_scatter_w4<h16_t>(NCLS) : plan_scatter_w4<float>(NCLS))) { hulc_set_error("hulc_k_plan_scatter_grad: form 1 (w4) serves the 16-bit types only"); return 1; }
    if (k_idx_out_of_range("hulc_k_plan_scatter_grad", idx, (long long)B * NCAT, NCLS, st)) return 1;
#define HULC_K_L(TT) launch_plan_scatter_grad<TT>(st, form == 1, (const TT*)dC, idx, B, NCAT, NCLS, H, KIN, dw, store)
    HULC_K_T("hulc_k_plan_scatter_grad", HULC_K_L);
#undef HULC_K_L
    return k_launched("hulc_k_plan_scatter_grad");
}

int k_normal_kl_sample(int t16, const float* pr_state, const float* pp_state, int B, int n, const float* eps_in, float* eps_out, float* plan_f, void* plan_t, float* kl_elem,
                       float* dpp, float* dpr, float w_pp, float w_pr, unsigned long long seed, const float* lscale, void* stream) {
    hipStream_t st = (hipStream_t)stream;
    if (B < 1 || n < 1 || (long long)B * n > (1ll << 29)) { hulc_set_error("hulc_k_normal_kl_sample: B=%d n=%d", B, n); return 1; }
    if (!pr_state || !eps_out || !plan_f || !plan_t || (pp_state && (!kl_elem || !dpp || !dpr))) { hulc_set_error("hulc_k_normal_kl_sample: null argument"); return 1; }
    if (k_misaligned(pr_state, 4) || k_misaligned(pp_state, 4) || k_misaligned(eps_in, 4) || k_misaligned(eps_out, 4) || k_misaligned(plan_f, 4) || k_misaligned(plan_t, t16 ? 2 : 4) ||
        k_misaligned(kl_elem, 4) || k_misaligned(dpp, 4) || k_misaligned(dpr, 4) || k_misaligned(lscale, 4)) { hulc_set_error("hulc_k_normal_kl_sample: a pointer is not aligned to its element type"); return 1; }
#define HULC_K_L(TT)                                                                                                                                               \
    hipLaunchKernelGGL((normal_kl_sample_kernel<TT>), dim3(cdiv((long long)B * n, 256)), dim3(256), 0, st, pr_state, pp_state, B, n, eps_in, eps_out, plan_f, (TT*)plan_t, kl_elem, \
                       dpp, dpr, w_pp, w_pr, seed, lscale)
    HULC_K_T("hulc_k_normal_kl_sample", HULC_K_L);
#undef HULC_K_L
    return k_launched("hulc_k_normal_kl_sample");
}

int k_normal_rsample_bwd(int t16, const float* dplan, const float* eps, const float* pr_state, const float* dpr_kl, int B, int n, void* out, void* stream) {
    hipStream_t st = (hipStream_t)stream;
    if (B < 1 || n < 1 || (long long)B * n > (1ll << 29)) { hulc_set_error("hulc_k_normal_rsample_bwd: B=%d n=%d", B, n); return 1; }
    if (!dplan || !eps || !pr_state || !dpr_kl || !out) { hulc_set_error("hulc_k_normal_rsample_bwd: null argument"); return 1; }
    if (k_misaligned(dplan, 4) || k_misaligned(eps, 4) || k_misaligned(pr_state, 4) || k_misaligned(dpr_kl, 4) || k_misaligned(out, t16 ? 2 : 4)) {
        hulc_set_error("hulc_k_normal_rsample_bwd: a pointer is not aligned to its element type"); return 1;
    }
#define HULC_K_L(TT) hipLaunchKernelGGL((normal_rsample_bwd_kernel<TT>), dim3(cdiv((long long)B * n, 256)), dim3(256), 0, st, dplan, eps, pr_state, dpr_kl, B, n, (TT*)out)
    HULC_K_T("hulc_k_normal_rsample_bwd", HULC_K_L);
#undef HULC_K_L
    return k_launched("hulc_k_normal_rsample_bwd");
}

int k_layernorm_fwd(int t16, const float* x, long long ldx, int rows, int n, const float* g, const float* b, void* out, long long ldo, float* out_f32, long long ldf, float* stats,
                    void* stream) {
    if (rows < 1 || n < 1 || n > 128 || ldx < n || (out && ldo < n) || (out_f32 && ldf < n) || rows > (1 << 24)) {
        hulc_set_error("hulc_k_layernorm_fwd: rows=%d n=%d ldx=%lld ldo=%lld ldf=%lld (need 1 <= n <= 128 and leading dimensions >= n)", rows, n, ldx, ldo, ldf); return 1;
    }
// ... 620 lines not shown
```

### hulc_amd/csrc/kernels.h

```cpp
#pragma once
#include "common.h"

namespace HULC_NS {

template <typename TS, typename TD>
__global__ void __launch_bounds__(256) cast_transpose_kernel(const TS* __restrict__ src, long long lds_, TD* __restrict__ dst,
                                                             long long ldd, TD* __restrict__ dstT, long long ldt, int R, int C) {
    __shared__ float tile[32][33];
    const int c0 = blockIdx.x * 32, r0 = blockIdx.y * 32;
    const int tx = threadIdx.x & 31, ty = threadIdx.x >> 5;
#pragma unroll
    for (int i = 0; i < 4; ++i) {
        const int r = r0 + ty + i * 8, c = c0 + tx;
        float v = 0.f;
        if (r < R && c < C) {
            v = to_f<TS>(src[(long long)r * lds_ + c]);
            if (dst) dst[(long long)r * ldd + c] = from_f<TD>(v);
        }
        tile[ty + i * 8][tx] = v;
    }
    if (!dstT) return;
    __syncthreads();
#pragma unroll
    for (int i = 0; i < 4; ++i) {
        const int c = c0 + ty + i * 8, r = r0 + tx;
        if (r < R && c < C) dstT[(long long)c * ldt + r] = from_f<TD>(tile[tx][ty + i * 8]);
    }
}

struct TrDesc { const void* src; void* dst; long long lds, ldt; int R, C, blk0, tiles_x; float* cs = nullptr; float* cs2 = nullptr;
                void* fr = nullptr; void* frT = nullptr; };
template <typename TS, typename TD>
__global__ void __launch_bounds__(256) batched_transpose_kernel(const TrDesc* __restrict__ desc, int ndesc) {
    __shared__ float tile[32][33];
    int lo = 0, hi = ndesc - 1;
    while (lo < hi) { const int mid = (lo + hi + 1) >> 1; if (desc[mid].blk0 <= (int)blockIdx.x) lo = mid; else hi = mid - 1; }
    const int d = lo;
    const TrDesc D = desc[d];
    const int b = blockIdx.x - D.blk0;
    const int c0 = (b % D.tiles_x) * 32, r0 = (b / D.tiles_x) * 32;
    const int tx = threadIdx.x & 31, ty = threadIdx.x >> 5;
    const TS* src = reinterpret_cast<const TS*>(D.src);
    TD* dst = reinterpret_cast<TD*>(D.dst);
#pragma unroll
    for (int i = 0; i < 4; ++i) {
        const int r = r0 + ty + i * 8, c = c0 + tx;
        tile[ty + i * 8][tx] = (r < D.R && c < D.C) ? to_f<TS>(src[(long long)r * D.lds + c]) : 0.f;
    }
    __syncthreads();
#pragma unroll
    for (int i = 0; i < 4; ++i) {
        const int c = c0 + ty + i * 8, r = r0 + tx;
        if (r < D.R && c < D.C) dst[(long long)c * D.ldt + r] = from_f<TD>(tile[tx][ty + i * 8]);
    }
// ... 126 lines not shown
    T* wd = reinterpret_cast<T*>(d.wd[c]);
    if (wf) {
        if (d.nhwc[c]) wf[(long long)o * (KH * KW * I) + (kh * KW + kw) * I + ci] = from_f<T>(v);
        else wf[idx] = from_f<T>(v);
    }
    if (wd) {
        const int ph = kh % S, a = kh / S, pw = kw % S, b = kw / S;
        const int TA = KH / S, TB = KW / S;
        const int zc = ph * S + pw;
        wd[((long long)zc * I + ci) * (TA * TB * O) + (a * TB + b) * O + o] = from_f<T>(v);
    }
}

__global__ void unpack_conv_wgrad_kernel(const float* __restrict__ part, int nsplit, long long slab, float* __restrict__ grad,
                                         int O, int I, int KH, int KW, int nhwc_fwd) {
    const int idx = (blockIdx.x * blockDim.x + threadIdx.x) * 4;
    const int total = O * I * KH * KW;
    if (idx >= total) return;
    const int per = (nsplit + gridDim.y - 1) / gridDim.y;
    const int z0 = blockIdx.y * per, z1 = min(nsplit, z0 + per);
    float4 s0 = make_float4(0.f, 0.f, 0.f, 0.f), s1 = s0, s2 = s0, s3 = s0;
    auto add4 = [](float4& a, const float4 b) { a.x += b.x; a.y += b.y; a.z += b.z; a.w += b.w; };
    int z = z0;
    for (; z + 7 < z1; z += 8) {
        float4 t[8];
#pragma unroll
        for (int u = 0; u < 8; ++u) t[u] = *reinterpret_cast<const float4*>(part + (long long)(z + u) * slab + idx);
        add4(s0, t[0]); add4(s1, t[1]); add4(s2, t[2]); add4(s3, t[3]);
        add4(s0, t[4]); add4(s1, t[5]); add4(s2, t[6]); add4(s3, t[7]);
    }
    for (; z + 3 < z1; z += 4) {
        const float4 a = *reinterpret_cast<const float4*>(part + (long long)z * slab + idx), b = *reinterpret_cast<const float4*>(part + (long long)(z + 1) * slab + idx);
        const float4 c = *reinterpret_cast<const float4*>(part + (long long)(z + 2) * slab + idx), d = *reinterpret_cast<const float4*>(part + (long long)(z + 3) * slab + idx);
        add4(s0, a); add4(s1, b); add4(s2, c); add4(s3, d);
    }
    for (; z < z1; ++z) add4(s0, *reinterpret_cast<const float4*>(part + (long long)z * slab + idx));
    const float v[4] = {(s0.x + s1.x) + (s2.x + s3.x), (s0.y + s1.y) + (s2.y + s3.y), (s0.z + s1.z) + (s2.z + s3.z), (s0.w + s1.w) + (s2.w + s3.w)};
#pragma unroll
    for (int e = 0; e < 4; ++e) {
        int dst = idx + e;
        if (nhwc_fwd) {
            int ci = dst % I, t = dst / I;
            int kw = t % KW; t /= KW;
            int kh = t % KH, o = t / KH;
            dst = ((o * I + ci) * KH + kh) * KW + kw;
        }
        if (gridDim.y > 1) unsafeAtomicAdd(grad + dst, v[e]);
        else grad[dst] += v[e];
    }
}

struct UnpackJob { const float* part; float* grad; long long slab; int nsplit, O, I, KH, KW, nhwc, blk0, ysplit; };
constexpr int UNPACK_MAX_JOBS = 12;
struct UnpackBatch { UnpackJob j[UNPACK_MAX_JOBS]; int n; };
__global__ void unpack_conv_wgrad_batched_kernel(UnpackBatch ub) {
    int k = 0;
    while (k + 1 < ub.n && (int)blockIdx.x >= ub.j[k + 1].blk0) ++k;
    const UnpackJob J = ub.j[k];
    const int idx = ((blockIdx.x - J.blk0) * blockDim.x + threadIdx.x) * 4;
    const int total = J.O * J.I * J.KH * J.KW;
    if (idx >= total) return;
    const int gy = J.ysplit > 0 ? J.ysplit : (int)gridDim.y;
    if ((int)blockIdx.y >= gy) return;
    const int per = (J.nsplit + gy - 1) / gy;
    const int z0 = blockIdx.y * per, z1 = min(J.nsplit, z0 + per);
    if (z0 >= z1) return;
    const float* part = J.part;
    const long long slab = J.slab;
    float4 s0 = make_float4(0.f, 0.f, 0.f, 0.f), s1 = s0, s2 = s0, s3 = s0;
    auto add4 = [](float4& a, const float4 b) { a.x += b.x; a.y += b.y; a.z += b.z; a.w += b.w; };
    int z = z0;
    for (; z + 7 < z1; z += 8) {
        float4 t[8];
#pragma unroll
        for (int u = 0; u < 8; ++u) t[u] = *reinterpret_cast<const float4*>(part + (long long)(z + u) * slab + idx);
        add4(s0, t[0]); add4(s1, t[1]); add4(s2, t[2]); add4(s3, t[3]);
        add4(s0, t[4]); add4(s1, t[5]); add4(s2, t[6]); add4(s3, t[7]);
    }
    for (; z + 3 < z1; z += 4) {
        const float4 a = *reinterpret_cast<const float4*>(part + (long long)z * slab + idx), b = *reinterpret_cast<const float4*>(part + (long long)(z + 1) * slab + idx);
        const float4 c = *reinterpret_cast<const float4*>(part + (long long)(z + 2) * slab + idx), d = *reinterpret_cast<const float4*>(part + (long long)(z + 3) * slab + idx);
        add4(s0, a); add4(s1, b); add4(s2, c); add4(s3, d);
    }
    for (; z < z1; ++z) add4(s0, *reinterpret_cast<const float4*>(part + (long long)z * slab + idx));
    const float v[4] = {(s0.x + s1.x) + (s2.x + s3.x), (s0.y + s1.y) + (s2.y + s3.y), (s0.z + s1.z) + (s2.z + s3.z), (s0.w + s1.w) + (s2.w + s3.w)};
    if (gy == 1 && !J.nhwc) {
        float4* g4 = reinterpret_cast<float4*>(J.grad + idx);
        float4 o = *g4;
        o.x += v[0]; o.y += v[1]; o.z += v[2]; o.w += v[3];
        *g4 = o;
        return;
    }
#pragma unroll
    for (int e = 0; e < 4; ++e) {
        int dst = idx + e;
        if (J.nhwc) {
            int ci = dst % J.I, t = dst / J.I;
            int kw = t % J.KW; t /= J.KW;
            int kh = t % J.KH, o = t / J.KH;
            dst = ((o * J.I + ci) * J.KH + kh) * J.KW + kw;
        }
        if (gy == 1) J.grad[dst] += v[e];
        else unsafeAtomicAdd(J.grad + dst, v[e]);
    }
}

template <typename TS, typename TD>
__global__ void permute_cols_kernel(const TS* __restrict__ src, TD* __restrict__ dst, int R, int CH, int P, int inverse,
// ... 1997 lines not shown
    { const f32x4nt t = __builtin_nontemporal_load(reinterpret_cast<const f32x4nt*>(a.g + i)); q.gg = make_float4(t[0], t[1], t[2], t[3]); }
    { const f32x4nt t = __builtin_nontemporal_load(reinterpret_cast<const f32x4nt*>(a.m + i)); q.mm = make_float4(t[0], t[1], t[2], t[3]); }
    { const f32x4nt t = __builtin_nontemporal_load(reinterpret_cast<const f32x4nt*>(a.v + i)); q.vv = make_float4(t[0], t[1], t[2], t[3]); }
}
DEVI void adam_finish4(const AdamArgs& a, float bc1, float bc2_sqrt, float gscale, long long i, AdamQuad& q, unsigned& lo, unsigned& hi, float vclip = 0.f) {
#pragma clang fp contract(off)
    typedef float f32x4nt __attribute__((ext_vector_type(4)));
    float4 &pp = q.pp, &gg = q.gg, &mm = q.mm, &vv = q.vv;
    float* P = &pp.x; float* G = &gg.x; float* Mv = &mm.x; float* V = &vv.x;
#pragma unroll
    for (int e = 0; e < 4; ++e) {
        float gr = G[e] * gscale;
        if (vclip > 0.f) gr = gr > vclip ? vclip : (gr < -vclip ? -vclip : gr);
        if (a.wd != 0.f) {
            if (a.decoupled) P[e] *= 1.f - a.lr * a.wd;
            else gr += a.wd * P[e];
        }
        Mv[e] = a.b1 * Mv[e] + (1.f - a.b1) * gr;
        V[e] = a.b2 * V[e] + (1.f - a.b2) * gr * gr;
        P[e] -= (a.lr / bc1) * Mv[e] / (sqrtf(V[e]) / bc2_sqrt + a.eps);
    }
    *reinterpret_cast<float4*>(a.p + i) = pp;
    lo = pack2h(pp.x, pp.y); hi = pack2h(pp.z, pp.w);
    if (a.shadow) *reinterpret_cast<uint2*>(a.shadow + i) = uint2{lo, hi};
    __builtin_nontemporal_store(f32x4nt{mm.x, mm.y, mm.z, mm.w}, reinterpret_cast<f32x4nt*>(a.m + i));
    __builtin_nontemporal_store(f32x4nt{vv.x, vv.y, vv.z, vv.w}, reinterpret_cast<f32x4nt*>(a.v + i));
}
DEVI void adam_update4(const AdamArgs& a, float bc1, float bc2_sqrt, float gscale, long long i, unsigned& lo, unsigned& hi, float vclip = 0.f) {
    AdamQuad q;
    adam_load4(a, i, q);
    adam_finish4(a, bc1, bc2_sqrt, gscale, i, q, lo, hi, vclip);
}
__global__ void adam_kernel(float* __restrict__ p, const float* __restrict__ g, float* __restrict__ m, float* __restrict__ v, long long n,
                            float lr, float b1, float b2, float eps, float bc1, float bc2_sqrt, float gscale, h16_t* __restrict__ shadow,
                            const ScalerState* __restrict__ ss = nullptr, float wd = 0.f, int decoupled = 0, const unsigned* __restrict__ skip = nullptr,
                            unsigned tag = 0, const ClipState* __restrict__ cs = nullptr) {
    if (skip && *skip == tag) return;
    if (ss) {
        if (ss->found_inf) return;
        gscale /= ss->scale;
        const float t = (float)(ss->steps + 1);
        bc1 = 1.f - powf(b1, t);
        bc2_sqrt = sqrtf(1.f - powf(b2, t));
    }
    float vclip;
    clip_read(cs, gscale, vclip);
    const AdamArgs a{p, g, m, v, lr, b1, b2, eps, bc1, bc2_sqrt, gscale, wd, decoupled, shadow, ss, skip, tag, cs};
    long long i = ((long long)blockIdx.x * blockDim.x + threadIdx.x) * 4;
    const long long stride = (long long)gridDim.x * blockDim.x * 4;
    for (; i + 3 < n; i += stride) { unsigned lo, hi; adam_update4(a, bc1, bc2_sqrt, gscale, i, lo, hi, vclip); }
}

constexpr int ADAM_CHUNK = 4096;
__global__ void __launch_bounds__(256) adam_tiled_kernel(AdamArgs a, const TrDesc* __restrict__ desc, const unsigned short* __restrict__ blk2desc, int ntile,
                                                         const long long* __restrict__ chunk_start, const int* __restrict__ chunk_n) {
    __shared__ __attribute__((aligned(16))) unsigned short tile[64][66];
    if (a.skip && *a.skip == a.tag) return;
    float gscale = a.gscale, bc1 = a.bc1, bc2_sqrt = a.bc2_sqrt;
    if (a.ss) {
        if (a.ss->found_inf) return;
        gscale /= a.ss->scale;
        const float t = (float)(a.ss->steps + 1);
        bc1 = 1.f - powf(a.b1, t);
        bc2_sqrt = sqrtf(1.f - powf(a.b2, t));
    }
    float vclip;
    clip_read(a.cs, gscale, vclip);
    const int tid = threadIdx.x;
    if ((int)blockIdx.x < ntile) {
        const TrDesc D = desc[blk2desc[blockIdx.x]];
        const int b = blockIdx.x - D.blk0;
        const int c0 = (b % D.tiles_x) * 64, r0 = (b / D.tiles_x) * 64;
        const long long off = reinterpret_cast<const h16_t*>(D.src) - a.shadow;
        const int cc = (tid & 15) * 4, c = c0 + cc;
        AdamQuad q[4];
#pragma unroll
        for (int ps = 0; ps < 4; ++ps) {
            const int r = r0 + ps * 16 + (tid >> 4);
            if (r < D.R && c < D.C) adam_load4(a, off + (long long)r * D.C + c, q[ps]);
        }
#pragma unroll
        for (int ps = 0; ps < 4; ++ps) {
            const int row = ps * 16 + (tid >> 4), r = r0 + row;
            unsigned lo = 0u, hi = 0u;
            if (r < D.R && c < D.C) adam_finish4(a, bc1, bc2_sqrt, gscale, off + (long long)r * D.C + c, q[ps], lo, hi, vclip);
            *reinterpret_cast<unsigned*>(&tile[row][cc]) = lo;
            *reinterpret_cast<unsigned*>(&tile[row][cc + 2]) = hi;
        }
        __syncthreads();
        if (D.fr) {
#pragma unroll
            for (int u = 0; u < 2; ++u) {
                const int q = tid + u * 256, row = q >> 3, c8 = q & 7;
                const int r = r0 + row, k = c0 + c8 * 8;
                if (r < D.R && k + 7 < D.C) {
                    uint4 v;
                    v.x = *reinterpret_cast<const unsigned*>(&tile[row][c8 * 8]); v.y = *reinterpret_cast<const unsigned*>(&tile[row][c8 * 8 + 2]);
                    v.z = *reinterpret_cast<const unsigned*>(&tile[row][c8 * 8 + 4]); v.w = *reinterpret_cast<const unsigned*>(&tile[row][c8 * 8 + 6]);
                    *reinterpret_cast<uint4*>(reinterpret_cast<h16_t*>(D.fr) + ((((long long)(r >> 4) * (D.C >> 5) + (k >> 5)) * 64 + ((k & 31) >> 3) * 16 + (r & 15)) << 3)) = v;
                }
            }
        }
        transpose_tile64_store(D, b, tile);
    } else {
        const int j = blockIdx.x - ntile;
        const long long start = chunk_start[j];
        const int n = chunk_n[j];
        for (int i = tid * 4; i + 3 < n; i += 1024) { unsigned lo, hi; adam_update4(a, bc1, bc2_sqrt, gscale, start + i, lo, hi, vclip); }
    }
}

__global__ void sgd_kernel(float* __restrict__ p, const float* __restrict__ g, float* __restrict__ buf, long long n, float lr, float momentum,
                           float dampening, float wd, int nesterov, int first, float gscale, h16_t* __restrict__ shadow,
                           const ScalerState* __restrict__ ss = nullptr, const unsigned* __restrict__ skip = nullptr, unsigned tag = 0,
                           const ClipState* __restrict__ cs = nullptr) {
    if (skip && *skip == tag) return;
    if (ss) {
        if (ss->found_inf) return;
        gscale /= ss->scale;
        first = ss->steps == 0;
    }
    float vclip;
    clip_read(cs, gscale, vclip);
    long long i = ((long long)blockIdx.x * blockDim.x + threadIdx.x) * 4;
    const long long stride = (long long)gridDim.x * blockDim.x * 4;
    for (; i + 3 < n; i += stride) {
        float4 pp = *reinterpret_cast<float4*>(p + i), gg = *reinterpret_cast<const float4*>(g + i), bb = make_float4(0.f, 0.f, 0.f, 0.f);
        if (momentum != 0.f && !first) bb = *reinterpret_cast<const float4*>(buf + i);
        float* P = &pp.x; float* G = &gg.x; float* Bf = &bb.x;
#pragma unroll
        for (int e = 0; e < 4; ++e) {
            float gr = G[e] * gscale;
            if (vclip > 0.f) gr = gr > vclip ? vclip : (gr < -vclip ? -vclip : gr);
            if (wd != 0.f) gr += wd * P[e];
            if (momentum != 0.f) {
                Bf[e] = first ? gr : momentum * Bf[e] + (1.f - dampening) * gr;
                gr = nesterov ? gr + momentum * Bf[e] : Bf[e];
            }
            P[e] -= lr * gr;
        }
        *reinterpret_cast<float4*>(p + i) = pp;
        if (momentum != 0.f) *reinterpret_cast<float4*>(buf + i) = bb;
        if (shadow) {
            uint2 o;
            o.x = pack2h(pp.x, pp.y);
            o.y = pack2h(pp.z, pp.w);
            *reinterpret_cast<uint2*>(shadow + i) = o;
        }
    }
}

template <typename T>
__global__ void gather_embg_kernel(const T* __restrict__ emb, T* __restrict__ out, int B, int S, int W = 64) {
    const int idx = blockIdx.x * blockDim.x + threadIdx.x;
    if (idx >= S * B * W) return;
    const int c = idx % W, r = idx / W;
    const int t = r / B, b = r % B;
    out[idx] = emb[((long long)b * S + t) * 128 + (128 - W) + c];
}
__global__ void pack_losses_kernel(float* __restrict__ l, float* __restrict__ out = nullptr) {
    l[4] = l[0] + l[1]; l[5] = l[1]; l[6] = l[0]; l[7] = l[2];
    if (out) { out[0] = l[4]; out[1] = l[5]; out[2] = l[6]; out[3] = l[7]; }
// ... 4 lines not shown
```

### hulc_amd/lib.py

```python
from __future__ import annotations

import ctypes as C
import os

_HERE = os.path.dirname(os.path.abspath(__file__))
LIB_PATH = os.path.join(_HERE, "csrc", "libhulc_hip.so")

KIND = {"hulc": 0, "gcbc": 1, "mcil": 2, "mcil_gru": 3}
DTYPE = {"fp32": 0, "bf16": 1, "fp16": 2}


class HulcConfig(C.Structure):
    _fields_ = [("kind", C.c_int32), ("dtype", C.c_int32), ("max_batch", C.c_int32), ("max_seq", C.c_int32),
                ("max_window", C.c_int32), ("use_clip", C.c_int32), ("kl_beta", C.c_float),
                ("kl_balancing_mix", C.c_float), ("dropout_p", C.c_float), ("num_classes", C.c_int32),
                ("gripper_alpha", C.c_float), ("log_scale_min", C.c_float), ("seed", C.c_uint64)]


class HulcBatch(C.Structure):
    _fields_ = [("B", C.c_int32), ("S", C.c_int32), ("is_lang", C.c_int32), ("rgb_static", C.c_void_p),
                ("rgb_gripper", C.c_void_p), ("actions", C.c_void_p), ("robot_obs", C.c_void_p), ("lang", C.c_void_p),
                ("plan_idx", C.c_void_p), ("aux_rows", C.c_void_p), ("n_aux", C.c_int32), ("step", C.c_uint64),
                ("frames_u8", C.c_int32), ("pad_static", C.c_int32), ("pad_gripper", C.c_int32), ("shift_static", C.c_void_p),
                ("shift_gripper", C.c_void_p), ("plan_eps", C.c_void_p), ("actions_absolute", C.c_int32), ("max_rel_pos", C.c_float),
                ("max_rel_orn", C.c_float), ("window_start", C.c_void_p), ("store_frames", C.c_int64), ("window_len", C.c_void_p),
                ("window_len_host", C.c_void_p)]


class HulcStoreTables(C.Structure):
    _fields_ = [("actions", C.c_void_p), ("robot_obs", C.c_void_p), ("lang", C.c_void_p), ("store_frames", C.c_int64), ("lang_rows", C.c_int32), ("absolute", C.c_int32)]


class HulcStageCopy(C.Structure):
    _fields_ = [("src", C.c_void_p), ("dst", C.c_void_p), ("bytes", C.c_int64)]


class HulcValNoise(C.Structure):
    _fields_ = [("plan_idx_pp", C.c_void_p), ("plan_idx_pr", C.c_void_p), ("u_mix_pp", C.c_void_p), ("u_act_pp", C.c_void_p),
                ("u_mix_pr", C.c_void_p), ("u_act_pr", C.c_void_p)]


class HulcRolloutObs(C.Structure):
    _fields_ = [("rgb_static", C.c_void_p), ("rgb_gripper", C.c_void_p), ("robot_obs_raw", C.c_void_p)]


class HulcRolloutEnvsObs(C.Structure):
    _fields_ = [("n", C.c_int32), ("slots", C.c_void_p), ("rgb_static", C.c_void_p), ("rgb_gripper", C.c_void_p), ("robot_obs_raw", C.c_void_p)]


class HulcOptim(C.Structure):
    _fields_ = [("kind", C.c_int32), ("lr", C.c_float), ("beta1", C.c_float), ("beta2", C.c_float), ("eps", C.c_float), ("weight_decay", C.c_float),
                ("momentum", C.c_float), ("dampening", C.c_float), ("nesterov", C.c_int32), ("step", C.c_int64), ("grad_scale", C.c_float)]


DECODER = {"logistic": 0, "deterministic": 1}
CRITERION = {"HuberLoss": 0, "MSELoss": 1}
OPTIM = {"adam": 0, "adamw": 1, "sgd": 2}
CLIP = {"off": 0, "norm": 1, "value": 2}


class HulcSbertConfig(C.Structure):
    _fields_ = [("layers", C.c_int32), ("hidden", C.c_int32), ("heads", C.c_int32), ("intermediate", C.c_int32), ("vocab", C.c_int32),
                ("max_position", C.c_int32), ("max_sentences", C.c_int32), ("max_tokens", C.c_int32), ("normalize", C.c_int32), ("ln_eps", C.c_float)]


class HulcConvJob(C.Structure):
    _fields_ = [("input", C.c_void_p), ("w", C.c_void_p), ("bias", C.c_void_p), ("out", C.c_void_p), ("bits", C.c_void_p),
                ("frames", C.c_int32), ("in_side", C.c_int32), ("out_side", C.c_int32)]


class HulcEncTailJob(C.Structure):
    _fields_ = [("x", C.c_void_p), ("W1", C.c_void_p), ("W2", C.c_void_p), ("b1", C.c_void_p), ("b2", C.c_void_p), ("lng", C.c_void_p), ("lnb", C.c_void_p),
                ("f1", C.c_void_p), ("f2", C.c_void_p), ("lnst", C.c_void_p), ("col0", C.c_int32)]


class HulcEncTailBwdJob(C.Structure):
    _fields_ = [("f2", C.c_void_p), ("lnst", C.c_void_p), ("lng", C.c_void_p), ("f1", C.c_void_p), ("W2t", C.c_void_p), ("W1t", C.c_void_p), ("xmask", C.c_void_p),
                ("dlng", C.c_void_p), ("dlnb", C.c_void_p), ("d_f2", C.c_void_p), ("d_f1", C.c_void_p), ("dx_f32", C.c_void_p), ("dx_t", C.c_void_p), ("col0", C.c_int32)]


class HulcTrLayerJob(C.Structure):
    _fields_ = [(n, C.c_void_p) for n in ("xin", "ln_g", "ln_b", "xf_out", "xt_out", "st_out", "Wqkv", "Wo", "W1", "W2", "bqkv", "bo", "b1", "b2", "n1g", "n1b",
                                          "qkv", "Pat", "ao", "y1", "st1", "x1t", "x1f", "hff", "y2")] + \
               [(n, C.c_uint64) for n in ("seed_att", "seed_o", "seed_h", "seed_y")]


class HulcTrFfnBwdJob(C.Structure):
    _fields_ = [(n, C.c_void_p) for n in ("dx", "y2", "st2", "n2g", "dg2", "db2", "W2t", "W1t", "hff", "dt_c", "dt_a", "part")] + [("seed_y", C.c_uint64)]


class HulcTrAttnBwdJob(C.Structure):
    _fields_ = [(n, C.c_void_p) for n in ("parts", "y1", "st1", "n1g", "dg1", "db1", "Wot", "Wint", "qkv", "Pat", "b_d", "b_b", "dy_f", "dx")] + \
               [("seed_o", C.c_uint64), ("seed_att", C.c_uint64)]


class HulcGemmEpiJob(C.Structure):
    _fields_ = [("A", C.c_void_p), ("B", C.c_void_p), ("M", C.c_int32), ("N", C.c_int32), ("K", C.c_int32), ("lda", C.c_int64), ("ldb", C.c_int64),
                ("ldc", C.c_int64), ("out_R1", C.c_int32), ("out_s0", C.c_int64), ("nsplit", C.c_int32), ("wfrag", C.c_int32),
                ("out", C.c_void_p), ("out_f32", C.c_int32), ("accumulate", C.c_int32), ("atomic", C.c_int32), ("z_stride", C.c_int64),
                ("bias", C.c_void_p), ("bias2", C.c_void_p), ("res", C.c_void_p), ("res_f32", C.c_int32), ("res_ld", C.c_int64), ("res_rowmod", C.c_int32),
                ("res_late", C.c_int32), ("mask", C.c_void_p), ("mask_tanh", C.c_int32), ("relu", C.c_int32), ("alpha", C.c_float), ("drop_p", C.c_float),
                ("drop_seed", C.c_uint64), ("out2", C.c_void_p), ("out2_lo", C.c_int64), ("out2_hi", C.c_int64), ("out2_mask", C.c_void_p),
                ("out2_relu", C.c_int32), ("generic_only", C.c_int32)]


GEMM_RAN = {"none": 0, "32": 1, "64": 2, "128": 3, "glds": 4, "skinny_router": 5, "skinny_reg": 6, "kchunk": 7, "splitk_64": 8, "splitk_128": 9, "group": 10, "pair": 11,
            "dual": 12}

EXPORTS = ["hulc_last_error", "hulc_ctx_create", "hulc_ctx_destroy", "hulc_set_stream", "hulc_workspace_bytes",
           "hulc_bind_params", "hulc_prepare_weights", "hulc_zero_grads", "hulc_flush_grads", "hulc_forward_loss", "hulc_forward_loss_pair", "hulc_backward", "hulc_backward_part",
           "hulc_adam_step", "hulc_optimizer_step", "hulc_comm_unique_id", "hulc_comm_prepare", "hulc_comm_init", "hulc_comm_destroy", "hulc_comm_buckets", "hulc_comm_stats", "hulc_comm_size", "hulc_comm_timeline", "hulc_allreduce_grads", "hulc_backward_allreduce", "hulc_scaler_enable", "hulc_scaler_get", "hulc_scaler_set", "hulc_grad_clip_set", "hulc_grad_norm_get", "hulc_validate", "hulc_store_gather", "hulc_store_stage", "hulc_store_stage_join", "hulc_store_stage_stats", "hulc_clip_gt_encode", "hulc_clip_gt_scores", "hulc_aux_heads_enable", "hulc_decoder_select", "hulc_aux_weights_set", "hulc_aux_losses_get", "hulc_rollout_reset", "hulc_rollout_plan", "hulc_rollout_act", "hulc_rollout_get_goal", "hulc_rollout_set_state", "hulc_rollout_envs_init", "hulc_rollout_envs_reset", "hulc_rollout_envs_plan", "hulc_rollout_envs_act", "hulc_rollout_envs_get_state", "hulc_rollout_envs_set_state", "hulc_sbert_create", "hulc_sbert_destroy", "hulc_sbert_set_stream", "hulc_sbert_bind", "hulc_sbert_encode", "hulc_set_kl_beta", "hulc_set_dropout", "hulc_set_option", "hulc_get_option", "hulc_timers_enable", "hulc_timers_read", "hulc_get_tensor", "hulc_get_plan_idx", "hulc_k_gemm_nt", "hulc_k_cast", "hulc_k_trread_probe", "hulc_k_conv_wgrad", "hulc_k_conv1_wgrad_u8", "hulc_k_conv1_interior_groups", "hulc_k_conv_tile", "hulc_k_camera_split", "hulc_k_conv_pair", "hulc_k_skinny", "hulc_k_attention", "hulc_k_rnn_persist", "hulc_k_rnn_persist_flag_words", "hulc_k_clip_loss", "hulc_k_clip_loss_fp32", "hulc_k_mia_head", "hulc_k_cosine_dist", "hulc_k_spatial_softmax64", "hulc_k_enc_tail_fwd", "hulc_k_enc_tail_bwd", "hulc_k_logistic_loss",
           "hulc_k_plan_kl_sample", "hulc_k_st_softmax_bwd", "hulc_k_plan_gather", "hulc_k_plan_scatter_grad", "hulc_k_normal_kl_sample", "hulc_k_normal_rsample_bwd",
           "hulc_k_layernorm_fwd", "hulc_k_layernorm_bwd", "hulc_k_layernorm_mean", "hulc_k_tr_layer_fwd", "hulc_k_tr_ffn_bwd", "hulc_k_tr_attn_bwd",
           "hulc_k_window_compact", "hulc_k_rows_expand", "hulc_k_rows_reduce", "hulc_k_gemm_epi", "hulc_k_gemm_multi", "hulc_k_gemm_pick", "hulc_k_gemm_wgrad_nsplit",
           "hulc_k_det_head_loss", "hulc_k_det_head_bwd", "hulc_k_det_head_act",
           "hulc_k_conv_wgrad_t", "hulc_k_conv1_wgrad_u8_t", "hulc_k_conv_tile_t", "hulc_k_conv_pair_t", "hulc_k_conv_plan"]

_lib = None


def load():
    global _lib
    if _lib is not None:
        return _lib
    path = os.environ.get("HULC_LIB_PATH") or LIB_PATH
    if not os.path.exists(path):
        raise RuntimeError(f"hulc_amd: {path} not built — run `python -c 'import __graft_entry__ as g; g.build()'`; "
                           "there is no CPU fallback for the product path")
    import torch
    lib = C.CDLL(path)
    lib.hulc_last_error.restype = C.c_char_p
    lib.hulc_workspace_bytes.restype = C.c_int64
    lib.hulc_ctx_create.argtypes = [C.POINTER(HulcConfig), C.POINTER(C.c_void_p)]
    lib.hulc_ctx_destroy.argtypes = [C.c_void_p]
    lib.hulc_set_stream.argtypes = [C.c_void_p, C.c_void_p]
    lib.hulc_workspace_bytes.argtypes = [C.c_void_p]
    lib.hulc_bind_params.argtypes = [C.c_void_p, C.c_void_p, C.c_void_p, C.c_void_p, C.c_void_p, C.c_int64, C.c_int32,
                                     C.POINTER(C.c_char_p), C.POINTER(C.c_int64), C.POINTER(C.c_int64)]
    lib.hulc_prepare_weights.argtypes = [C.c_void_p]
    lib.hulc_zero_grads.argtypes = [C.c_void_p]
    if os.environ.get("HULC_LIB_PATH") and not hasattr(lib, "hulc_flush_grads"):
        lib.hulc_zero_grads.argtypes = [C.c_void_p]
    else:
        lib.hulc_flush_grads.argtypes = [C.c_void_p]
    lib.hulc_forward_loss.argtypes = [C.c_void_p, C.POINTER(HulcBatch), C.c_float, C.c_float, C.c_void_p, C.c_int32]
    lib.hulc_forward_loss_pair.argtypes = [C.c_void_p, C.POINTER(HulcBatch), C.POINTER(HulcBatch), C.c_float, C.c_float, C.c_void_p, C.c_int32]
    lib.hulc_backward.argtypes = [C.c_void_p]
    lib.hulc_backward_part.argtypes = [C.c_void_p, C.c_int32]
    lib.hulc_adam_step.argtypes = [C.c_void_p, C.c_float, C.c_float, C.c_float, C.c_float, C.c_int64, C.c_float]
    lib.hulc_optimizer_step.argtypes = [C.c_void_p, C.POINTER(HulcOptim)]
    lib.hulc_comm_unique_id.argtypes = [C.c_void_p, C.c_int64]
    lib.hulc_comm_prepare.argtypes = [C.c_void_p]
    lib.hulc_comm_init.argtypes = [C.c_void_p, C.c_void_p, C.c_int32, C.c_int32]
    lib.hulc_comm_destroy.argtypes = [C.c_void_p]
    lib.hulc_comm_buckets.argtypes = [C.c_void_p, C.POINTER(C.c_int64), C.POINTER(C.c_int64), C.c_int32]
    lib.hulc_comm_stats.argtypes = [C.c_void_p, C.POINTER(C.c_int64), C.POINTER(C.c_double)]
    if hasattr(lib, "hulc_comm_size") or not os.environ.get("HULC_LIB_PATH"):
        lib.hulc_comm_size.argtypes = [C.c_void_p, C.POINTER(C.c_int32), C.POINTER(C.c_int32)]
    lib.hulc_comm_timeline.argtypes = [C.c_void_p, C.POINTER(C.c_double), C.c_int32, C.POINTER(C.c_double)]
    lib.hulc_allreduce_grads.argtypes = [C.c_void_p, C.c_int32]
    lib.hulc_backward_allreduce.argtypes = [C.c_void_p, C.c_int32]
    lib.hulc_scaler_enable.argtypes = [C.c_void_p, C.c_float, C.c_float, C.c_float, C.c_int32]
    lib.hulc_scaler_get.argtypes = [C.c_void_p, C.POINTER(C.c_float), C.POINTER(C.c_int32), C.POINTER(C.c_int64), C.POINTER(C.c_int32), C.POINTER(C.c_int64)]
    lib.hulc_scaler_set.argtypes = [C.c_void_p, C.c_float, C.c_int32, C.c_int64]
    if hasattr(lib, "hulc_grad_clip_set") or not os.environ.get("HULC_LIB_PATH"):
        lib.hulc_grad_clip_set.argtypes = [C.c_void_p, C.c_int32, C.c_float, C.c_int32]
        lib.hulc_grad_norm_get.argtypes = [C.c_void_p, C.POINTER(C.c_float), C.POINTER(C.c_float), C.c_void_p, C.c_int64]
    lib.hulc_clip_gt_encode.argtypes = [C.c_void_p, C.c_void_p, C.c_int32, C.c_int32]
# ... 54 lines not shown
    if hasattr(lib, "hulc_k_clip_loss") or not os.environ.get("HULC_LIB_PATH"):
        for f in (lib.hulc_k_clip_loss, lib.hulc_k_clip_loss_fp32):
            f.argtypes = [C.c_void_p, C.c_void_p, C.c_int32, C.c_void_p, C.c_float, C.c_void_p, C.c_void_p, C.c_void_p, C.c_void_p, C.c_void_p]
        lib.hulc_k_mia_head.argtypes = [C.c_void_p, C.c_void_p, C.c_int32, C.c_void_p, C.c_void_p, C.c_void_p, C.c_void_p, C.c_float, C.c_void_p, C.c_void_p, C.c_void_p,
                                        C.c_int32, C.c_void_p, C.c_void_p, C.c_void_p, C.c_void_p, C.c_void_p]
        lib.hulc_k_cosine_dist.argtypes = [C.c_void_p, C.c_void_p, C.c_int32, C.c_int32, C.c_float, C.c_void_p, C.c_void_p, C.c_void_p]
    lib.hulc_k_attention.argtypes = [C.c_int32, C.c_void_p, C.c_void_p, C.c_void_p, C.c_void_p, C.c_void_p, C.c_int32, C.c_int32, C.c_float, C.c_uint64, C.c_void_p]
    if hasattr(lib, "hulc_k_enc_tail_fwd") or not os.environ.get("HULC_LIB_PATH"):
        lib.hulc_k_spatial_softmax64.argtypes = [C.c_int32, C.c_void_p, C.c_int32, C.c_int32, C.c_int32, C.c_void_p, C.c_void_p, C.c_void_p, C.c_void_p, C.c_void_p]
        lib.hulc_k_enc_tail_fwd.argtypes = [C.c_int32, C.c_int32, C.c_int32, C.POINTER(HulcEncTailJob), C.POINTER(HulcEncTailJob), C.c_void_p, C.c_void_p, C.c_int32,
                                            C.c_float, C.c_uint64, C.c_void_p, C.c_void_p, C.c_void_p, C.c_void_p, C.c_void_p]
        lib.hulc_k_enc_tail_bwd.argtypes = [C.c_int32, C.c_int32, C.c_int32, C.POINTER(HulcEncTailBwdJob), C.POINTER(HulcEncTailBwdJob), C.c_void_p, C.c_void_p]
        lib.hulc_k_logistic_loss.argtypes = [C.c_int32, C.c_int32, C.c_void_p, C.c_int32, C.c_void_p, C.c_void_p, C.c_int32, C.c_int32, C.c_int32, C.c_int32, C.c_int32,
                                             C.c_float, C.c_float, C.c_int32, C.c_int32, C.c_float, C.c_void_p, C.c_void_p, C.c_void_p, C.c_void_p, C.c_void_p]
    if hasattr(lib, "hulc_k_layernorm_bwd") or not os.environ.get("HULC_LIB_PATH"):
        P, I, F, U, Q = C.c_void_p, C.c_int32, C.c_float, C.c_uint64, C.c_int64
        lib.hulc_k_plan_kl_sample.argtypes = [P, P, I, I, I, P, P, P, P, P, P, F, F, U, P, P]
        lib.hulc_k_st_softmax_bwd.argtypes = [I, P, P, P, P, I, I, P, P, P, P]
        lib.hulc_k_plan_gather.argtypes = [I, P, P, I, I, I, I, P, P, P, P, P, I, I, P, I, I, P, P]
        lib.hulc_k_plan_scatter_grad.argtypes = [I, I, P, P, I, I, I, I, I, P, I, P]
        lib.hulc_k_normal_kl_sample.argtypes = [I, P, P, I, I, P, P, P, P, P, P, P, F, F, U, P, P]
        lib.hulc_k_normal_rsample_bwd.argtypes = [I, P, P, P, P, I, I, P, P]
        lib.hulc_k_layernorm_fwd.argtypes = [I, P, Q, I, I, P, P, P, Q, P, Q, P, P]
        lib.hulc_k_layernorm_bwd.argtypes = [I, P, Q, P, Q, P, P, I, I, P, Q, I, P, Q, P, P, F, U, I, F, I, Q, P, P]
        lib.hulc_k_layernorm_mean.argtypes = [I, P, I, I, I, P, P, P, P, P, P]
    if hasattr(lib, "hulc_k_tr_layer_fwd") or not os.environ.get("HULC_LIB_PATH"):
        lib.hulc_k_tr_layer_fwd.argtypes = [C.c_int32, C.POINTER(HulcTrLayerJob), C.c_int32, C.c_int32, C.c_int32, C.c_float, C.c_void_p]
        lib.hulc_k_tr_ffn_bwd.argtypes = [C.c_int32, C.POINTER(HulcTrFfnBwdJob), C.c_int32, C.c_int32, C.c_int32, C.c_float, C.c_float, C.c_void_p]
        lib.hulc_k_tr_attn_bwd.argtypes = [C.c_int32, C.POINTER(HulcTrAttnBwdJob), C.c_int32, C.c_int32, C.c_int32, C.c_int64, C.c_float, C.c_void_p]
    if hasattr(lib, "hulc_k_rows_reduce") or not os.environ.get("HULC_LIB_PATH"):
        P, I, Q = C.c_void_p, C.c_int32, C.c_int64
        lib.hulc_k_window_compact.argtypes = [P, P, P, I, I, I, Q, P, P, P, P, P, P]
        lib.hulc_k_rows_expand.argtypes = [I, P, P, P, I, I, I, P, P]
        lib.hulc_k_rows_reduce.argtypes = [P, P, P, I, I, I, P, P]
    if hasattr(lib, "hulc_k_gemm_epi") or not os.environ.get("HULC_LIB_PATH"):
        I, Q, PI = C.c_int32, C.c_int64, C.POINTER(C.c_int32)
        lib.hulc_k_gemm_epi.argtypes = [I, C.POINTER(HulcGemmEpiJob), I, PI, C.c_void_p]
        lib.hulc_k_gemm_multi.argtypes = [I, I, C.POINTER(HulcGemmEpiJob), I, I, PI, C.c_void_p]
        lib.hulc_k_gemm_pick.argtypes = [I, I, I, I, Q, Q, PI, PI]
        lib.hulc_k_gemm_wgrad_nsplit.argtypes = [I, I, I, I, PI, PI]
    if hasattr(lib, "hulc_decoder_select") or not os.environ.get("HULC_LIB_PATH"):
        P, I, F = C.c_void_p, C.c_int32, C.c_float
        lib.hulc_decoder_select.argtypes = [P, I, I]
        lib.hulc_k_det_head_loss.argtypes = [I, P, P, P, P, P, I, I, I, I, F, P, P, P, P, P]
        lib.hulc_k_det_head_bwd.argtypes = [I, P, P, P, I, I, P, P, P, P, P]
        lib.hulc_k_det_head_act.argtypes = [I, P, P, P, P, I, P, P]
    if hasattr(lib, "hulc_k_conv_plan") or not os.environ.get("HULC_LIB_PATH"):
        P, I, PI = C.c_void_p, C.c_int32, C.POINTER(C.c_int32)
        lib.hulc_k_conv_wgrad_t.argtypes = [I, I, P, P, P, P, I, I, PI, P]
        lib.hulc_k_conv1_wgrad_u8_t.argtypes = [I, P, P, I, P, P, P, I, I, I, I, PI, P]
        lib.hulc_k_conv_tile_t.argtypes = [I, I, P, P, P, P, P, P, I, I, I, I, I, P]
        lib.hulc_k_conv_pair_t.argtypes = [I, I, C.POINTER(HulcConvJob), C.POINTER(HulcConvJob), I, I, PI, P]
        lib.hulc_k_conv_plan.argtypes = [I, I, I, I, I, PI, PI, PI, PI]
    _lib = lib
    return lib


def check(rc: int):
    if rc != 0:
        raise RuntimeError("libhulc_hip: " + load().hulc_last_error().decode("utf-8", "replace"))
```

### include/hulc_hip.h

```cpp
#ifndef HULC_HIP_H
#define HULC_HIP_H
#include <stdint.h>

#ifdef __cplusplus
extern "C" {
#endif

typedef struct hulc_ctx hulc_ctx;

enum { HULC_KIND_HULC = 0, HULC_KIND_GCBC = 1, HULC_KIND_MCIL = 2, HULC_KIND_MCIL_GRU = 3 };
enum { HULC_DTYPE_F32 = 0, HULC_DTYPE_BF16 = 1, HULC_DTYPE_F16 = 2 };

typedef struct hulc_config {
    int32_t kind;
    int32_t dtype;
    int32_t max_batch;
    int32_t max_seq;
    int32_t max_window;
    int32_t use_clip;
    float kl_beta;
    float kl_balancing_mix;
    float dropout_p;
    int32_t num_classes;
    float gripper_alpha;
// ... 196 lines not shown
int hulc_k_conv1_wgrad_u8_t(int32_t dtype, const void* X, const int32_t* shifts, int32_t pad, const void* dY, float* dw_out, float* db_out, int32_t Nf, int32_t IH, int32_t form,
                            int32_t fold, int32_t* slabs, void* hip_stream);
int hulc_k_conv_tile_t(int32_t dtype, int32_t mode, const void* img, const void* w, const float* bias, const void* mask, void* out, uint32_t* bits1_out, int32_t Nf, int32_t IMH,
                       int32_t OUTH, int32_t relu, int32_t wgs, void* hip_stream);
int hulc_k_conv_pair_t(int32_t dtype, int32_t stage, const hulc_conv_job* a, const hulc_conv_job* b, int32_t wg_a, int32_t wg_b, int32_t* slabs, void* hip_stream);
int hulc_k_conv_plan(int32_t form, int32_t frames, int32_t in_side, int32_t out_side, int32_t wgs, int32_t* nbands, int32_t* rows_per_band, int32_t* frames_per_band, int32_t* items);
int hulc_k_skinny(const void* A, const void* W, void* out, int32_t M, int32_t N, int32_t K, int32_t variant, void* hip_stream);
int hulc_k_rnn_persist(void* X, const void* W, const void* res, const void* mask, int32_t B, int32_t S, int32_t q0, int32_t dq, int32_t act,
                       uint32_t* flags, uint32_t* err, uint32_t launch_index, void* hip_stream);
int32_t hulc_k_rnn_persist_flag_words(void);
int hulc_k_trread_probe(const int32_t* elem_index_per_lane , uint16_t* out , void* hip_stream);
int hulc_k_cast(int32_t dtype, const float* src, void* dst, int64_t n, void* hip_stream);
int hulc_k_attention(int32_t variant, const float* qkv, float* P, float* ao, const float* dao, float* dqkv, int32_t B, int32_t S,
                     float drop_p, uint64_t seed, void* hip_stream);

int hulc_k_clip_loss(const float* img, const float* txt, int32_t n, const float* logit_scale, float w, float* loss_out, float* dimg, float* dtxt,
                     float* dlogit_scale, void* hip_stream);
int hulc_k_clip_loss_fp32(const float* img, const float* txt, int32_t n, const float* logit_scale, float w, float* loss_out, float* dimg, float* dtxt,
                          float* dlogit_scale, void* hip_stream);
int hulc_k_mia_head(const float* img, const float* txt, int32_t n, const float* W0, const float* b0, const float* W1, const float* b1, float w, float* loss_out,
                    float* dimg, float* dtxt, int32_t accum, float* dW0, float* db0, float* dW1, float* db1, void* hip_stream);
int hulc_k_cosine_dist(const float* pred, const float* tgt, int32_t n, int32_t D, float w, float* loss_out, float* dpred, void* hip_stream);

int hulc_k_spatial_softmax64(int32_t dtype, const void* f, int32_t H, int32_t W, int32_t Nf, void* out, float* stats, const float* dout, void* df, void* hip_stream);
typedef struct hulc_enc_tail_job {
    const void* x; const void* W1; const void* W2; const float* b1; const float* b2; const float* lng; const float* lnb;
    void* f1; float* f2; float* lnst;
    int32_t col0;
} hulc_enc_tail_job;
int hulc_k_enc_tail_fwd(int32_t dtype, int32_t Nf, int32_t ldemb, const hulc_enc_tail_job* a, const hulc_enc_tail_job* b, void* emb, const float* pos, int32_t S,
                        float drop_p, uint64_t seed, float* xf, void* xt, float* z0, float* z1, void* hip_stream);
typedef struct hulc_enc_tail_bwd_job {
    const float* f2; const float* lnst; const float* lng; const void* f1; const void* W2t; const void* W1t; const void* xmask;
    float* dlng; float* dlnb; void* d_f2; void* d_f1; float* dx_f32; void* dx_t;
    int32_t col0;
} hulc_enc_tail_bwd_job;
int hulc_k_enc_tail_bwd(int32_t dtype, int32_t Nf, int32_t ldemb, const hulc_enc_tail_bwd_job* a, const hulc_enc_tail_bwd_job* b, const float* demb, void* hip_stream);
int hulc_k_logistic_loss(int32_t dtype, int32_t wide, const float* heads, int32_t ldh, const float* actions, const float* robot_obs, int32_t B, int32_t S,
                         int32_t n_mix, int32_t n_dim, int32_t num_classes, float log_scale_min, float gripper_alpha, int32_t gripper_control,
                         int32_t discrete_gripper, float grad_scale, const float* lscale, float* row_loss, float* a_tcp_out, void* dheads, void* hip_stream);

int hulc_k_det_head_loss(int32_t dtype, const void* H1, const void* W, const float* bias, const float* actions, const float* robot_obs, int32_t B, int32_t S,
                         int32_t criterion, int32_t frame, float grad_scale, const float* lscale, float* row_loss, float* pred, float* dpre, void* hip_stream);
int hulc_k_det_head_bwd(int32_t dtype, const float* dpre, const void* W, const void* H1, int32_t B, int32_t S, void* dH1, void* dZ1, float* dW, float* db,
                        void* hip_stream);
int hulc_k_det_head_act(int32_t dtype, const void* h1, const void* W, const float* bias, const float* robot_obs, int32_t n, float* out, void* hip_stream);

int hulc_k_plan_kl_sample(const float* pr_logits, const float* pp_logits, int32_t B, int32_t NCAT, int32_t NCLS, const int32_t* idx_in, int32_t* idx_out, float* probs,
                          float* kl_cat, float* dpp, float* dpr, float w_pp, float w_pr, uint64_t seed, const float* lscale, void* hip_stream);
int hulc_k_st_softmax_bwd(int32_t dtype, const float* probs, const float* dplan, const float* dpr_kl, const float* dpp_kl, int32_t rows, int32_t NCLS, float* out,
                          void* out_t, void* dpp_t, void* hip_stream);
int hulc_k_plan_gather(int32_t dtype, const void* w_t, const int32_t* idx, int32_t B, int32_t NCAT, int32_t NCLS, int32_t H, const float* b1, const float* b2, float* out,
                       const void* emb, void* embg, int32_t S, int32_t W, const void* goal, int32_t G, int32_t grow0, void* cb, void* hip_stream);
int hulc_k_plan_scatter_grad(int32_t dtype, int32_t form, const void* dC, const int32_t* idx, int32_t B, int32_t NCAT, int32_t NCLS, int32_t H, int32_t KIN, float* dw,
                             int32_t store, void* hip_stream);
int hulc_k_normal_kl_sample(int32_t dtype, const float* pr_state, const float* pp_state, int32_t B, int32_t n, const float* eps_in, float* eps_out, float* plan_f, void* plan_t,
                            float* kl_elem, float* dpp, float* dpr, float w_pp, float w_pr, uint64_t seed, const float* lscale, void* hip_stream);
int hulc_k_normal_rsample_bwd(int32_t dtype, const float* dplan, const float* eps, const float* pr_state, const float* dpr_kl, int32_t B, int32_t n, void* out,
                              void* hip_stream);
int hulc_k_layernorm_fwd(int32_t dtype, const float* x, int64_t ldx, int32_t rows, int32_t n, const float* g, const float* b, void* out, int64_t ldo, float* out_f32,
                         int64_t ldf, float* stats, void* hip_stream);
int hulc_k_layernorm_bwd(int32_t dtype, const float* dy, int64_t lddy, const float* x, int64_t ldx, const float* stats, const float* g, int32_t rows, int32_t n, float* dx_f32,
                         int64_t ldd, int32_t accumulate, void* dx_t, int64_t ldt, float* dg, float* db, float drop_p, uint64_t seed, int32_t bcast_rows, float bcast_div,
                         int32_t dy_parts, int64_t dy_part_stride, float* scratch, void* hip_stream);
int hulc_k_layernorm_mean(int32_t dtype, const float* x, int32_t B, int32_t S, int32_t n, const float* g, const float* b, float* stats, void* out, float* yout,
                          void* hip_stream);
int hulc_k_window_compact(const int64_t* window_start, const int32_t* lens, const int32_t* off, int32_t off_base, int32_t B, int32_t S, int64_t store_frames,
                          const int32_t* shift_static, const int32_t* shift_gripper, int64_t* frame_out, int32_t* shift_static_out, int32_t* shift_gripper_out,
                          void* hip_stream);
int hulc_k_rows_expand(int32_t elem_bytes, const void* src, const int32_t* lens, const int32_t* off, int32_t B, int32_t S, int32_t n, void* dst, void* hip_stream);
int hulc_k_rows_reduce(const float* src, const int32_t* lens, const int32_t* off, int32_t B, int32_t S, int32_t n, float* dst, void* hip_stream);

typedef struct hulc_tr_layer_job {
    const float* xin; const float* ln_g; const float* ln_b; float* xf_out; void* xt_out; float* st_out;
    const void* Wqkv; const void* Wo; const void* W1; const void* W2;
    const float* bqkv; const float* bo; const float* b1; const float* b2; const float* n1g; const float* n1b;
    void* qkv; float* Pat; void* ao; float* y1; float* st1; void* x1t; float* x1f; void* hff; float* y2;
    uint64_t seed_att, seed_o, seed_h, seed_y;
} hulc_tr_layer_job;
int hulc_k_tr_layer_fwd(int32_t dtype, const hulc_tr_layer_job* job, int32_t B, int32_t S, int32_t ln_in, float dp, void* hip_stream);
typedef struct hulc_tr_ffn_bwd_job {
    const float* dx; const float* y2; const float* st2; const float* n2g; float* dg2; float* db2;
    const void* W2t; const void* W1t; const void* hff; void* dt_c; void* dt_a; float* part;
    uint64_t seed_y;
} hulc_tr_ffn_bwd_job;
int hulc_k_tr_ffn_bwd(int32_t dtype, const hulc_tr_ffn_bwd_job* job, int32_t B, int32_t S, int32_t bcast, float bdiv, float dp, void* hip_stream);
typedef struct hulc_tr_attn_bwd_job {
    const float* parts; const float* y1; const float* st1; const float* n1g; float* dg1; float* db1;
    const void* Wot; const void* Wint; const void* qkv; const float* Pat; void* b_d; void* b_b; float* dy_f; float* dx;
    uint64_t seed_o, seed_att;
} hulc_tr_attn_bwd_job;
int hulc_k_tr_attn_bwd(int32_t dtype, const hulc_tr_attn_bwd_job* job, int32_t B, int32_t S, int32_t nparts, int64_t part_stride, float dp, void* hip_stream);

typedef struct hulc_gemm_epi_job {
    const void* A; const void* B; int32_t M, N, K; int64_t lda, ldb;
    int64_t ldc; int32_t out_R1; int64_t out_s0;
    int32_t nsplit, wfrag;
    void* out; int32_t out_f32, accumulate, atomic; int64_t z_stride;
    const float* bias; const float* bias2;
    const void* res; int32_t res_f32; int64_t res_ld; int32_t res_rowmod, res_late;
    const void* mask; int32_t mask_tanh, relu; float alpha, drop_p; uint64_t drop_seed;
    void* out2; int64_t out2_lo, out2_hi; const void* out2_mask; int32_t out2_relu, generic_only;
} hulc_gemm_epi_job;
enum { HULC_GEMM_RAN_NONE = 0, HULC_GEMM_RAN_32 = 1, HULC_GEMM_RAN_64 = 2, HULC_GEMM_RAN_128 = 3, HULC_GEMM_RAN_GLDS = 4, HULC_GEMM_RAN_SKINNY_ROUTER = 5, HULC_GEMM_RAN_SKINNY_REG = 6,
       HULC_GEMM_RAN_KCHUNK = 7, HULC_GEMM_RAN_SPLITK_64 = 8, HULC_GEMM_RAN_SPLITK_128 = 9, HULC_GEMM_RAN_GROUP = 10, HULC_GEMM_RAN_PAIR = 11, HULC_GEMM_RAN_DUAL = 12 };
int hulc_k_gemm_epi(int32_t dtype, const hulc_gemm_epi_job* job, int32_t kernel, int32_t* ran, void* hip_stream);
// ... 9 lines not shown
```

Before: 21850 windows/s.

## Fuse weight repacking into Adam step and gradient zeroing into wgrad unpack

The tiled Adam kernel now writes the bf16 packed and transposed layouts of the conv, fc7 and head weights directly, so the separate pack pass in the next forward is skipped when both the shadow and the packs are fresh. Pack-job chunks are sorted first and mapped to per-chunk job descriptors. Separately, the final conv wgrad unpack launch also zeroes the stale lazy gradient ranges in extra blocks, which replaces a separate sweep. This removes kernel launches and redundant weight reads, at the cost of scattered stores inside Adam and more intricate freshness bookkeeping.

```diff
diff --git a/hulc_amd/csrc/capi.hip b/hulc_amd/csrc/capi.hip
--- a/hulc_amd/csrc/capi.hip
+++ b/hulc_amd/csrc/capi.hip
@@ -392,6 +392,16 @@
 int hulc_k_plan_gather(int32_t dtype, const void* w_t, const int32_t* idx, int32_t B, int32_t NCAT, int32_t NCLS, int32_t H, const float* b1, const float* b2, float* out,
                        const void* emb, void* embg, int32_t S, int32_t W, const void* goal, int32_t G, int32_t grow0, void* cb, void* stream) {
     HULC_K_ANY("hulc_k_plan_gather", k_plan_gather, w_t, idx, B, NCAT, NCLS, H, b1, b2, out, emb, embg, S, W, goal, G, grow0, cb, stream);
+}
+int hulc_k_unpack_sweep(const float* part, float* grad, int32_t O, int32_t I, int32_t KH, int32_t KW, int32_t nhwc, int32_t nsplit, int32_t ysplit, int32_t yparts, int32_t nzero,
+                        float* const* zp, const int64_t* zn, int32_t zblocks, void* stream) {
+    return hulc_bf16::k_unpack_sweep(part, grad, O, I, KH, KW, nhwc, nsplit, ysplit, yparts, nzero, zp, (const long long*)zn, zblocks, stream);
+}
+int hulc_k_adam_pack(int32_t dtype, float* p, const float* g, float* m, float* v, void* shadow, int64_t numel, const hulc_adam_pack_job* jobs, int32_t n_jobs, float lr,
+                     float beta1, float beta2, float eps, int64_t step, float weight_decay, int32_t decoupled, void* stream) {
+    if (dtype == HULC_DTYPE_F16) return hulc_f16::k_adam_pack(p, g, m, v, shadow, (long long)numel, jobs, n_jobs, lr, beta1, beta2, eps, (long long)step, weight_decay, decoupled, stream);
+    if (dtype != HULC_DTYPE_BF16) { hulc_set_error("hulc_k_adam_pack: dtype %d (the tiled optimizer step serves the 16-bit engines: BF16 or F16)", (int)dtype); return 1; }
+    return hulc_bf16::k_adam_pack(p, g, m, v, shadow, (long long)numel, jobs, n_jobs, lr, beta1, beta2, eps, (long long)step, weight_decay, decoupled, stream);
 }
 int hulc_k_plan_scatter_grad(int32_t dtype, int32_t form, const void* dC, const int32_t* idx, int32_t B, int32_t NCAT, int32_t NCLS, int32_t H, int32_t KIN, float* dw,
                              int32_t store, void* stream) {
diff --git a/hulc_amd/csrc/engine.h b/hulc_amd/csrc/engine.h
--- a/hulc_amd/csrc/engine.h
+++ b/hulc_amd/csrc/engine.h
@@ -87,6 +87,9 @@
     struct TrTable { TrDesc* desc = nullptr; unsigned short* b2d = nullptr; int blocks = 0, n = 0; };
     TrTable tr_adam, tr_rest;
     long long* adam_chunk_start = nullptr; int* adam_chunk_n = nullptr; int adam_chunks = 0;
+    AdamPackJob* adam_pack_jobs = nullptr; int* adam_chunk_job = nullptr; int adam_pack_chunks = 0;
+    bool pack_by_adam = false;
+    bool packs_fresh = false;
     bool adam_fuse_tr = true;
     void set_adam_fuse(bool on) override { adam_fuse_tr = on; }
     bool frag_by_adam = false;
@@ -109,7 +112,8 @@
     void adam_tables_build() {
         tr_table_free(tr_adam); tr_table_free(tr_rest); rest_by_pack = false; frag_by_adam = false;
         if (adam_chunk_start) { hipFree(adam_chunk_start); adam_chunk_start = nullptr; } if (adam_chunk_n) { hipFree(adam_chunk_n); adam_chunk_n = nullptr; }
-        adam_chunks = 0;
+        if (adam_pack_jobs) { hipFree(adam_pack_jobs); adam_pack_jobs = nullptr; } if (adam_chunk_job) { hipFree(adam_chunk_job); adam_chunk_job = nullptr; }
+        adam_chunks = 0; pack_by_adam = false; packs_fresh = false;
         if (std::is_same<T, float>::value || !wshadow || (numel & 3)) return;
         std::vector<TrDesc> fused, rest;
         std::vector<std::pair<long long, long long>> rng;
@@ -122,9 +126,42 @@
         std::sort(rng.begin(), rng.end());
         for (size_t i = 0; i + 1 < rng.size(); ++i) if (rng[i].second > rng[i + 1].first) return;
         if (fused.empty() || fused.size() > 65535) return;
-        std::vector<long long> cs; std::vector<int> cn;
+        std::vector<long long> cs; std::vector<int> cn, cj;
+        std::vector<AdamPackJob> pjobs;
+        {
+            auto job = [&](const float* src, long long n, int kind) -> AdamPackJob* {
+                AdamPackJob J{}; J.base = src - P; J.n = (int)n; J.kind = kind; pjobs.push_back(J); return &pjobs.back(); };
+            pjobs.reserve(16);
+            bool ok = true;
+            for (EncW* e : {&encS, &encG})
+                for (ConvW* c : {&e->c1, &e->c2, &e->c3}) {
+                    if (!c->W32) { ok = false; continue; }
+                    AdamPackJob* J = job(c->W32, (long long)c->O * c->I * c->KH * c->KW, 0);
+                    J->a[0] = c->O; J->a[1] = c->I; J->a[2] = c->KH; J->a[3] = c->S; J->a[4] = c->nhwc; J->d0 = c->Wf; J->d1 = c->nhwc ? c->Wd : nullptr;
+                    if (c->KH != c->KW) ok = false;
+                }
+            if (encG.fc7.W32 && encG.fc7.W) { AdamPackJob* J = job(encG.fc7.W32, 128ll * 3136, 1); J->a[0] = 128; J->a[1] = 64; J->a[2] = 49; J->d0 = encG.fc7.W; J->d1 = encG.fc7.Wt; }
+            else ok = false;
+            int row0 = 0;
+            for (int i = 0; i < 4; ++i) {
+                if (head_rows[i] > 0) {
+                    if (!head_w32[i] || !head_b32[i] || !wheads || !bheads) { ok = false; break; }
+                    AdamPackJob* J = job(head_w32[i], (long long)head_rows[i] * HID, 2); J->a[0] = row0; J->a[1] = HID; J->a[2] = NHEAD; J->d0 = wheads; J->d1 = wheadsT;
+                    J = job(head_b32[i], head_rows[i], 3); J->a[0] = row0; J->f0 = bheads;
+                }
+                row0 += head_rows[i];
+            }
+            std::sort(pjobs.begin(), pjobs.end(), [](const AdamPackJob& a, const AdamPackJob& b) { return a.base < b.base; });
+            auto end4 = [](const AdamPackJob& J) { return (J.base + J.n + 3) / 4 * 4; };
+            for (size_t i = 0; i < pjobs.size() && ok; ++i) {
+                const AdamPackJob& J = pjobs[i];
+                if (J.base < 0 || (J.base & 3) || end4(J) > numel || (i + 1 < pjobs.size() && end4(J) > pjobs[i + 1].base)) ok = false;
+                for (auto& r : rng) if (J.base < r.second && end4(J) > r.first) ok = false;
+            }
+            if (!ok) pjobs.clear();
+        }
         long long pos = 0;
-        auto cover = [&](long long lo, long long hi) { for (long long x = lo; x < hi; x += ADAM_CHUNK) { cs.push_back(x); cn.push_back((int)std::min<long long>(ADAM_CHUNK, hi - x)); } };
+        auto cover = [&](long long lo, long long hi) { adam_cover_range(lo, hi, pjobs, cs, cn, cj); };
         for (auto& r : rng) { cover(pos, r.first); pos = r.second; }
         cover(pos, numel);
         if (!tr_table_build(tr_adam, fused) || !tr_table_build(tr_rest, rest)) { tr_table_free(tr_adam); tr_table_free(tr_rest); return; }
@@ -135,11 +172,27 @@
             const bool hd = d.src == (const void*)wheads && d.dst == (void*)wheadsT && d.R == NHEAD && d.C == HID && d.ldt == NHEAD;
             if (!f7 && !hd) rest_by_pack = false;
         }
+        {
+            std::vector<size_t> ord(cs.size());
+            for (size_t i = 0; i < ord.size(); ++i) ord[i] = i;
+            std::stable_sort(ord.begin(), ord.end(), [&](size_t a, size_t b) { return (cj[a] >= 0) > (cj[b] >= 0); });
+            std::vector<long long> cs2; std::vector<int> cn2, cj2;
+            for (size_t i : ord) { cs2.push_back(cs[i]); cn2.push_back(cn[i]); cj2.push_back(cj[i]); }
+            cs.swap(cs2); cn.swap(cn2); cj.swap(cj2);
+            adam_pack_chunks = 0;
+            for (int j : cj) if (j >= 0) ++adam_pack_chunks;
+        }
         adam_chunks = (int)cs.size();
         if (adam_chunks) {
             if (hipMalloc((void**)&adam_chunk_start, sizeof(long long) * cs.size()) != hipSuccess || hipMalloc((void**)&adam_chunk_n, sizeof(int) * cn.size()) != hipSuccess) { tr_table_free(tr_adam); tr_table_free(tr_rest); adam_chunks = 0; return; }
             hipMemcpy(adam_chunk_start, cs.data(), sizeof(long long) * cs.size(), hipMemcpyHostToDevice);
             hipMemcpy(adam_chunk_n, cn.data(), sizeof(int) * cn.size(), hipMemcpyHostToDevice);
+            if (!pjobs.empty() && hipMalloc((void**)&adam_pack_jobs, sizeof(AdamPackJob) * pjobs.size()) == hipSuccess && hipMalloc((void**)&adam_chunk_job, sizeof(int) * cj.size()) == hipSuccess) {
+                if (!rest_by_pack) for (AdamPackJob& J : pjobs) if (J.kind == 1 || J.kind == 2) J.d1 = nullptr;
+                hipMemcpy(adam_pack_jobs, pjobs.data(), sizeof(AdamPackJob) * pjobs.size(), hipMemcpyHostToDevice);
+                hipMemcpy(adam_chunk_job, cj.data(), sizeof(int) * cj.size(), hipMemcpyHostToDevice);
+                pack_by_adam = true;
+            }
         }
     }
 
@@ -189,7 +242,7 @@
         KIN = dec_plan + DE + GOAL;
         maxB = cfg.max_batch; maxS = cfg.max_seq; maxN = maxB * maxS;
     }
-    ~Engine() override { for (void* p : allocs) hipFree(p); if (rp_err_host) hipHostFree((void*)rp_err_host); if (blk2desc_dev) hipFree(blk2desc_dev); if (trdesc_dev) hipFree(trdesc_dev); tr_table_free(tr_adam); tr_table_free(tr_rest); if (adam_chunk_start) hipFree(adam_chunk_start); if (adam_chunk_n) hipFree(adam_chunk_n); gn_free(); if (clip_state) hipFree(clip_state); if (env_rows_host) hipHostFree(env_rows_host); }
+    ~Engine() override { for (void* p : allocs) hipFree(p); if (rp_err_host) hipHostFree((void*)rp_err_host); if (blk2desc_dev) hipFree(blk2desc_dev); if (trdesc_dev) hipFree(trdesc_dev); tr_table_free(tr_adam); tr_table_free(tr_rest); if (adam_chunk_start) hipFree(adam_chunk_start); if (adam_chunk_n) hipFree(adam_chunk_n); if (adam_pack_jobs) hipFree(adam_pack_jobs); if (adam_chunk_job) hipFree(adam_chunk_job); gn_free(); if (clip_state) hipFree(clip_state); if (env_rows_host) hipHostFree(env_rows_host); }
     int64_t workspace_bytes() const override { return ws_bytes; }
     void set_kl_beta(float b) override { cfg.kl_beta = b; }
     void set_dropout(float p) override { cfg.dropout_p = p; }
@@ -703,7 +756,9 @@
         if constexpr (!std::is_same<T, float>::value) {
             if (!shadow_fresh) hipLaunchKernelGGL((cast_kernel<float, T>), dim3(2048), dim3(256), 0, st, P, wshadow, (long long)numel);
         }
-        {
+        const bool packed = shadow_fresh && packs_fresh;
+        packs_fresh = false;
+        if (!packed) {
             ConvPackBatch d;
             int k = 0, blk = 0;
             for (EncW* e : {&encS, &encG})
@@ -948,8 +1003,9 @@
         else if (adam_fuse_tr && tr_adam.n && shadow) {
             AdamArgs a{P, G, AM, AV, lr, b1, b2, eps, (float)bc1d, (float)sqrt(bc2d), gscale, o.weight_decay, (int)(o.kind == HULC_OPT_ADAMW), shadow, (const ScalerState*)scaler, (const unsigned*)rp_skip, tag, cs};
             hipLaunchKernelGGL(adam_tiled_kernel, dim3(tr_adam.blocks + adam_chunks), dim3(256), 0, st, a, (const TrDesc*)tr_adam.desc, (const unsigned short*)tr_adam.b2d, tr_adam.blocks,
-                               (const long long*)adam_chunk_start, (const int*)adam_chunk_n);
-            tr_fresh = true;
+                               (const long long*)adam_chunk_start, (const int*)adam_chunk_n, (const AdamPackJob*)(pack_by_adam ? adam_pack_jobs : nullptr),
+                               (const int*)(pack_by_adam ? adam_chunk_job : nullptr), pack_by_adam ? adam_pack_chunks : 0);
+            tr_fresh = true; packs_fresh = pack_by_adam;
         } else
             hipLaunchKernelGGL(adam_kernel, dim3(2048), dim3(256), 0, st, P, G, AM, AV, (long long)numel, lr, b1, b2, eps, (float)bc1d, (float)sqrt(bc2d), gscale,
                                shadow, (const ScalerState*)scaler, o.weight_decay, (int)(o.kind == HULC_OPT_ADAMW), (const unsigned*)rp_skip, tag, cs);
diff --git a/hulc_amd/csrc/engine_backward.inc b/hulc_amd/csrc/engine_backward.inc
--- a/hulc_amd/csrc/engine_backward.inc
+++ b/hulc_amd/csrc/engine_backward.inc
@@ -429,7 +429,7 @@
             if (ragged()) launch_rows_reduce(st, demb, rg_lens(), rg_off(), B, S, EMB, demb_c);
             if (tail_fused) enc_tail_bwd_both(Nenc);
             enc_bwd_both(src, pair ? src2 : nullptr, Nenc, tail_fused);
-            flush_unpacks();
+            flush_unpacks(true);
         }
         if (bucket_ready(4)) return 1;
         lazy_sweep(0, numel, st);
diff --git a/hulc_amd/csrc/engine_encoders.inc b/hulc_amd/csrc/engine_encoders.inc
--- a/hulc_amd/csrc/engine_encoders.inc
+++ b/hulc_amd/csrc/engine_encoders.inc
@@ -234,9 +234,21 @@
         unpack_blocks += cdiv((int)slab, 1024); part_cur += nsplit * slab;
         return slabs;
     }
-    void flush_unpacks() {
+    void flush_unpacks(bool sweep = false) {
         constexpr int yparts = 8;
-        if (unpack_jobs.n > 0) hipLaunchKernelGGL(unpack_conv_wgrad_batched_kernel, dim3(unpack_blocks, yparts), dim3(256), 0, st, unpack_jobs);
+        int zblocks = 0;
+        unpack_jobs.nzero = 0;
+        if (sweep && unpack_jobs.n > 0) {
+            long long n4 = 0;
+            for (auto& z : this->lazy)
+                if (z.stale && unpack_jobs.nzero < UNPACK_MAX_ZERO) {
+                    unpack_jobs.zp[unpack_jobs.nzero] = this->G + z.off; unpack_jobs.zn[unpack_jobs.nzero] = z.n; ++unpack_jobs.nzero;
+                    n4 += z.n / 4; z.stale = false;
+                }
+            if (unpack_jobs.nzero) zblocks = (int)std::max<long long>(1, std::min<long long>(128, cdiv(n4, 256ll * yparts * 4)));
+            unpack_jobs.zblk0 = unpack_blocks;
+        }
+        if (unpack_jobs.n > 0) hipLaunchKernelGGL(unpack_conv_wgrad_batched_kernel, dim3(unpack_blocks + zblocks, yparts), dim3(256), 0, st, unpack_jobs);
         unpack_jobs.n = 0; part_cur = 0; unpack_blocks = 0;
     }
     bool tail_fc7_done = false;
diff --git a/hulc_amd/csrc/iengine.h b/hulc_amd/csrc/iengine.h
--- a/hulc_amd/csrc/iengine.h
+++ b/hulc_amd/csrc/iengine.h
@@ -168,6 +168,10 @@
                          void* out_t, void* dpp_t, void* stream);                                                                               \
     int k_plan_gather(int t16, const void* w_t, const int* idx, int B, int NCAT, int NCLS, int H, const float* b1, const float* b2, float* out,   \
                       const void* emb, void* embg, int S, int W, const void* goal, int G, int grow0, void* cb, void* stream);                     \
+    int k_unpack_sweep(const float* part, float* grad, int O, int I, int KH, int KW, int nhwc, int nsplit, int ysplit, int yparts, int nzero,      \
+                       float* const* zp, const long long* zn, int zblocks, void* stream);                                                           \
+    int k_adam_pack(float* p, const float* g, float* m, float* v, void* shadow, long long numel, const hulc_adam_pack_job* jobs, int n_jobs, float lr,   \
+                    float b1, float b2, float eps, long long step, float wd, int decoupled, void* stream);                                            \
     int k_plan_scatter_grad(int t16, int form, const void* dC, const int* idx, int B, int NCAT, int NCLS, int H, int KIN, float* dw, int store,   \
                             void* stream);                                                                                                      \
     int k_normal_kl_sample(int t16, const float* pr_state, const float* pp_state, int B, int n, const float* eps_in, float* eps_out, float* plan_f, \
diff --git a/hulc_amd/csrc/k_entries.h b/hulc_amd/csrc/k_entries.h
--- a/hulc_amd/csrc/k_entries.h
+++ b/hulc_amd/csrc/k_entries.h
@@ -225,6 +225,69 @@
     HULC_K_T("hulc_k_plan_gather", HULC_K_L);
 #undef HULC_K_L
     return k_launched("hulc_k_plan_gather");
+}
+
+int k_unpack_sweep(const float* part, float* grad, int O, int I, int KH, int KW, int nhwc, int nsplit, int ysplit, int yparts, int nzero, float* const* zp, const long long* zn,
+                   int zblocks, void* stream) {
+    hipStream_t st = (hipStream_t)stream;
+    const long long slab = (long long)O * I * KH * KW;
+    if (O < 1 || I < 1 || KH < 1 || KW < 1 || slab > (1ll << 28) || (slab & 3) || nsplit < 1 || yparts < 1 || yparts > 64 || ysplit < 0 || ysplit > yparts) {
+        hulc_set_error("hulc_k_unpack_sweep: O=%d I=%d KH=%d KW=%d nsplit=%d ysplit=%d yparts=%d (need a slab of a multiple of 4 elements, nsplit >= 1, 0 <= ysplit <= yparts <= 64)", O, I, KH, KW, nsplit, ysplit, yparts); return 1;
+    }
+    if (nzero < 0 || nzero > UNPACK_MAX_ZERO || (nzero > 0 && (!zp || !zn || zblocks < 1 || zblocks > 1024))) { hulc_set_error("hulc_k_unpack_sweep: nzero=%d zblocks=%d (need 0 <= nzero <= %d; with ranges: zp, zn and 1 <= zblocks <= 1024)", nzero, zblocks, UNPACK_MAX_ZERO); return 1; }
+    if (!part || !grad || k_misaligned(part, 16) || k_misaligned(grad, 16)) { hulc_set_error("hulc_k_unpack_sweep: part and grad must be given and 16-byte aligned"); return 1; }
+    UnpackBatch ub{};
+    UnpackJob& U = ub.j[0];
+    U.part = part; U.grad = grad; U.slab = slab; U.nsplit = nsplit; U.O = O; U.I = I; U.KH = KH; U.KW = KW; U.nhwc = nhwc ? 1 : 0; U.blk0 = 0; U.ysplit = ysplit;
+    ub.n = 1;
+    const int blocks = cdiv(slab, 1024);
+    for (int s = 0; s < nzero; ++s) {
+        if (!zp[s] || k_misaligned(zp[s], 16) || zn[s] < 0 || (zn[s] & 3)) { hulc_set_error("hulc_k_unpack_sweep: zero range %d must be 16-byte aligned and a multiple of 4 elements", s); return 1; }
+        ub.zp[s] = zp[s]; ub.zn[s] = zn[s];
+    }
+    ub.nzero = nzero; ub.zblk0 = blocks;
+    hipLaunchKernelGGL(unpack_conv_wgrad_batched_kernel, dim3(blocks + (nzero ? zblocks : 0), yparts), dim3(256), 0, st, ub);
+    return k_launched("hulc_k_unpack_sweep");
+}
+
+int k_adam_pack(float* p, const float* g, float* m, float* v, void* shadow, long long numel, const hulc_adam_pack_job* jobs, int n_jobs, float lr, float b1, float b2, float eps,
+                long long step, float wd, int decoupled, void* stream) {
+    hipStream_t st = (hipStream_t)stream;
+    if (!p || !g || !m || !v || !shadow || numel < 4 || (numel & 3) || numel > (1ll << 30) || n_jobs < 0 || n_jobs > 64 || (n_jobs && !jobs) || step < 1) {
+        hulc_set_error("hulc_k_adam_pack: null argument, numel=%lld (a multiple of 4), n_jobs=%d (<= 64) or step=%lld (>= 1)", numel, n_jobs, step); return 1; }
+    if (k_misaligned(p, 16) || k_misaligned(g, 16) || k_misaligned(m, 16) || k_misaligned(v, 16) || k_misaligned(shadow, 8)) { hulc_set_error("hulc_k_adam_pack: p, g, m, v must be 16-byte aligned, shadow 8"); return 1; }
+    std::vector<AdamPackJob> pj;
+    for (int i = 0; i < n_jobs; ++i) {
+        const hulc_adam_pack_job& s = jobs[i];
+        AdamPackJob J{}; J.base = s.base; J.n = s.n; J.kind = s.kind; for (int k = 0; k < 5; ++k) J.a[k] = s.a[k]; J.d0 = s.d0; J.d1 = s.d1; J.f0 = s.f0;
+        bool bad = s.base < 0 || (s.base & 3) || s.n < 1 || (s.base + s.n + 3) / 4 * 4 > numel || s.kind < 0 || s.kind > 3;
+        if (!bad && s.kind == 0) bad = s.a[0] < 1 || s.a[1] < 1 || s.a[2] < 1 || s.a[3] < 1 || (s.a[2] % s.a[3]) || (long long)s.a[0] * s.a[1] * s.a[2] * s.a[2] != s.n;
+        if (!bad && s.kind == 1) bad = s.a[0] < 1 || s.a[1] < 1 || s.a[2] < 1 || (long long)s.a[0] * s.a[1] * s.a[2] != s.n || !s.d0;
+        if (!bad && s.kind == 2) bad = s.a[0] < 0 || s.a[1] < 1 || (s.n % s.a[1]) || !s.d0 || (s.d1 && s.a[2] < s.a[0] + s.n / s.a[1]);
+        if (!bad && s.kind == 3) bad = s.a[0] < 0 || !s.f0;
+        if (bad || k_misaligned(s.d0, 2) || k_misaligned(s.d1, 2) || k_misaligned(s.f0, 4)) { hulc_set_error("hulc_k_adam_pack: job %d: range, kind, shape or pointer out of range", i); return 1; }
+        pj.push_back(J);
+    }
+    std::sort(pj.begin(), pj.end(), [](const AdamPackJob& a, const AdamPackJob& b) { return a.base < b.base; });
+    for (size_t i = 0; i + 1 < pj.size(); ++i) if ((pj[i].base + pj[i].n + 3) / 4 * 4 > pj[i + 1].base) { hulc_set_error("hulc_k_adam_pack: jobs overlap"); return 1; }
+    std::vector<long long> cs; std::vector<int> cn, cj;
+    adam_cover_range(0, numel, pj, cs, cn, cj);
+    long long* d_cs = nullptr; int *d_cn = nullptr, *d_cj = nullptr; AdamPackJob* d_pj = nullptr;
+    auto fre = [&]() { hipFree(d_cs); hipFree(d_cn); hipFree(d_cj); hipFree(d_pj); };
+    if (hipMalloc((void**)&d_cs, sizeof(long long) * cs.size()) != hipSuccess || hipMalloc((void**)&d_cn, sizeof(int) * cn.size()) != hipSuccess ||
+        hipMalloc((void**)&d_cj, sizeof(int) * cj.size()) != hipSuccess || hipMalloc((void**)&d_pj, sizeof(AdamPackJob) * std::max<size_t>(pj.size(), 1)) != hipSuccess) {
+        fre(); hulc_set_error("hulc_k_adam_pack: hipMalloc failed"); return 1; }
+    hipMemcpy(d_cs, cs.data(), sizeof(long long) * cs.size(), hipMemcpyHostToDevice); hipMemcpy(d_cn, cn.data(), sizeof(int) * cn.size(), hipMemcpyHostToDevice);
+    hipMemcpy(d_cj, cj.data(), sizeof(int) * cj.size(), hipMemcpyHostToDevice);
+    if (!pj.empty()) hipMemcpy(d_pj, pj.data(), sizeof(AdamPackJob) * pj.size(), hipMemcpyHostToDevice);
+    const double bc1d = 1.0 - pow((double)b1, (double)step), bc2d = 1.0 - pow((double)b2, (double)step);
+    AdamArgs a{p, g, m, v, lr, b1, b2, eps, (float)bc1d, (float)sqrt(bc2d), 1.f, wd, decoupled ? 1 : 0, (h16_t*)shadow, nullptr, nullptr, 0u, nullptr};
+    hipLaunchKernelGGL(adam_tiled_kernel, dim3((unsigned)cs.size()), dim3(256), 0, st, a, (const TrDesc*)nullptr, (const unsigned short*)nullptr, 0, (const long long*)d_cs, (const int*)d_cn,
+                       (const AdamPackJob*)d_pj, (const int*)d_cj);
+    const hipError_t e1 = hipGetLastError(), e2 = hipStreamSynchronize(st);
+    fre();
+    if (e1 != hipSuccess || e2 != hipSuccess) { hulc_set_error("hulc_k_adam_pack: %s", hipGetErrorString(e1 != hipSuccess ? e1 : e2)); return 1; }
+    return 0;
 }
 
 int k_plan_scatter_grad(int t16, int form, const void* dC, const int* idx, int B, int NCAT, int NCLS, int H, int KIN, float* dw, int store, void* stream) {
diff --git a/hulc_amd/csrc/kernels.h b/hulc_amd/csrc/kernels.h
--- a/hulc_amd/csrc/kernels.h
+++ b/hulc_amd/csrc/kernels.h
@@ -1,5 +1,7 @@
 #pragma once
 #include "common.h"
+#include <algorithm>
+#include <vector>
 
 namespace HULC_NS {
 
@@ -232,8 +234,20 @@
 
 struct UnpackJob { const float* part; float* grad; long long slab; int nsplit, O, I, KH, KW, nhwc, blk0, ysplit; };
 constexpr int UNPACK_MAX_JOBS = 12;
-struct UnpackBatch { UnpackJob j[UNPACK_MAX_JOBS]; int n; };
+constexpr int UNPACK_MAX_ZERO = 6;
+struct UnpackBatch { UnpackJob j[UNPACK_MAX_JOBS]; int n; int nzero, zblk0; float* zp[UNPACK_MAX_ZERO]; long long zn[UNPACK_MAX_ZERO]; };
 __global__ void unpack_conv_wgrad_batched_kernel(UnpackBatch ub) {
+    if (ub.nzero > 0 && (int)blockIdx.x >= ub.zblk0) {
+        const long long nthr = (long long)(gridDim.x - ub.zblk0) * gridDim.y * blockDim.x;
+        const long long t0 = ((long long)blockIdx.y * (gridDim.x - ub.zblk0) + (blockIdx.x - ub.zblk0)) * blockDim.x + threadIdx.x;
+        const float4 z = {0.f, 0.f, 0.f, 0.f};
+        for (int s = 0; s < ub.nzero; ++s) {
+            float4* __restrict__ d = reinterpret_cast<float4*>(ub.zp[s]);
+            const long long n4 = ub.zn[s] >> 2;
+            for (long long i = t0; i < n4; i += nthr) d[i] = z;
+        }
+        return;
+    }
     int k = 0;
     while (k + 1 < ub.n && (int)blockIdx.x >= ub.j[k + 1].blk0) ++k;
     const UnpackJob J = ub.j[k];
@@ -2337,8 +2351,43 @@
 }
 
 constexpr int ADAM_CHUNK = 4096;
+struct AdamPackJob { long long base; int n, kind; int a[5]; void* d0; void* d1; float* f0; };
+DEVI void adam_pack_store(const AdamPackJob& J, int idx, h16_t h, float f) {
+    if (idx >= J.n) return;
+    h16_t* d0 = reinterpret_cast<h16_t*>(J.d0);
+    h16_t* d1 = reinterpret_cast<h16_t*>(J.d1);
+    if (J.kind == 0) {
+        const int O = J.a[0], I = J.a[1], KH = J.a[2], KW = J.a[2], S = J.a[3];
+        int kw = idx % KW, t = idx / KW;
+        int kh = t % KH; t /= KH;
+        int ci = t % I, o = t / I;
+        if (d0) {
+            if (J.a[4]) d0[(long long)o * (KH * KW * I) + (kh * KW + kw) * I + ci] = h;
+            else d0[idx] = h;
+        }
+        if (d1) {
+            const int ph = kh % S, a = kh / S, pw = kw % S, b = kw / S;
+            const int TA = KH / S, TB = KW / S;
+            const int zc = ph * S + pw;
+            d1[((long long)zc * I + ci) * (TA * TB * O) + (a * TB + b) * O + o] = h;
+        }
+    } else if (J.kind == 1) {
+        const int R7 = J.a[0], CH7 = J.a[1], P7 = J.a[2];
+        const int c = idx % (CH7 * P7);
+        const long long r = idx / (CH7 * P7);
+        const int ch = c / P7, pp = c % P7;
+        d0[r * (CH7 * P7) + pp * CH7 + ch] = h;
+        if (d1) d1[(long long)(pp * CH7 + ch) * R7 + r] = h;
+    } else if (J.kind == 2) {
+        const int HID = J.a[1];
+        const long long pidx = (long long)J.a[0] * HID + idx;
+        d0[pidx] = h;
+        if (d1) d1[(long long)(idx % HID) * J.a[2] + pidx / HID] = h;
+    } else J.f0[J.a[0] + idx] = f;
+}
 __global__ void __launch_bounds__(256) adam_tiled_kernel(AdamArgs a, const TrDesc* __restrict__ desc, const unsigned short* __restrict__ blk2desc, int ntile,
-                                                         const long long* __restrict__ chunk_start, const int* __restrict__ chunk_n) {
+                                                         const long long* __restrict__ chunk_start, const int* __restrict__ chunk_n,
+                                                         const AdamPackJob* __restrict__ pack_jobs = nullptr, const int* __restrict__ chunk_job = nullptr, int nfirst = 0) {
     __shared__ __attribute__((aligned(16))) unsigned short tile[64][66];
     if (a.skip && *a.skip == a.tag) return;
     float gscale = a.gscale, bc1 = a.bc1, bc2_sqrt = a.bc2_sqrt;
@@ -2352,9 +2401,10 @@
     float vclip;
     clip_read(a.cs, gscale, vclip);
     const int tid = threadIdx.x;
-    if ((int)blockIdx.x < ntile) {
-        const TrDesc D = desc[blk2desc[blockIdx.x]];
-        const int b = blockIdx.x - D.blk0;
+    if ((int)blockIdx.x >= nfirst && (int)blockIdx.x < nfirst + ntile) {
+        const int tb = blockIdx.x - nfirst;
+        const TrDesc D = desc[blk2desc[tb]];
+        const int b = tb - D.blk0;
         const int c0 = (b % D.tiles_x) * 64, r0 = (b / D.tiles_x) * 64;
         const long long off = reinterpret_cast<const h16_t*>(D.src) - a.shadow;
         const int cc = (tid & 15) * 4, c = c0 + cc;
@@ -2388,11 +2438,35 @@
         }
         transpose_tile64_store(D, b, tile);
     } else {
-        const int j = blockIdx.x - ntile;
+        const int j = (int)blockIdx.x < nfirst ? blockIdx.x : blockIdx.x - ntile;
         const long long start = chunk_start[j];
         const int n = chunk_n[j];
+        const int pj = chunk_job ? chunk_job[j] : -1;
+        if (pj >= 0) {
+            const AdamPackJob J = pack_jobs[pj];
+            for (int i = tid * 4; i + 3 < n; i += 1024) {
+                unsigned lo, hi;
+                AdamQuad q;
+                adam_load4(a, start + i, q);
+                adam_finish4(a, bc1, bc2_sqrt, gscale, start + i, q, lo, hi, vclip);
+                const int e0 = (int)(start + i - J.base);
+                adam_pack_store(J, e0, (h16_t)(lo & 0xffffu), q.pp.x); adam_pack_store(J, e0 + 1, (h16_t)(lo >> 16), q.pp.y);
+                adam_pack_store(J, e0 + 2, (h16_t)(hi & 0xffffu), q.pp.z); adam_pack_store(J, e0 + 3, (h16_t)(hi >> 16), q.pp.w);
+            }
+            return;
+        }
         for (int i = tid * 4; i + 3 < n; i += 1024) { unsigned lo, hi; adam_update4(a, bc1, bc2_sqrt, gscale, start + i, lo, hi, vclip); }
     }
+}
+
+static inline void adam_cover_range(long long lo, long long hi, const std::vector<AdamPackJob>& jobs, std::vector<long long>& cs, std::vector<int>& cn, std::vector<int>& cj) {
+    auto cover1 = [&](long long a, long long b, int j) { for (long long x = a; x < b; x += ADAM_CHUNK) { cs.push_back(x); cn.push_back((int)std::min<long long>(ADAM_CHUNK, b - x)); cj.push_back(j); } };
+    for (size_t i = 0; i < jobs.size() && lo < hi; ++i) {
+        const long long jl = jobs[i].base, jh = (jobs[i].base + jobs[i].n + 3) / 4 * 4;
+        if (jl < lo || jh > hi) continue;
+        cover1(lo, jl, -1); cover1(jl, jh, (int)i); lo = jh;
+    }
+    cover1(lo, hi, -1);
 }
 
 __global__ void sgd_kernel(float* __restrict__ p, const float* __restrict__ g, float* __restrict__ buf, long long n, float lr, float momentum,
diff --git a/hulc_amd/lib.py b/hulc_amd/lib.py
--- a/hulc_amd/lib.py
+++ b/hulc_amd/lib.py
@@ -27,6 +27,10 @@
                 ("window_len_host", C.c_void_p)]
 
 
+class HulcAdamPackJob(C.Structure):
+    _fields_ = [("base", C.c_int64), ("n", C.c_int32), ("kind", C.c_int32), ("a", C.c_int32 * 5), ("d0", C.c_void_p), ("d1", C.c_void_p), ("f0", C.c_void_p)]
+
+
 class HulcStoreTables(C.Structure):
     _fields_ = [("actions", C.c_void_p), ("robot_obs", C.c_void_p), ("lang", C.c_void_p), ("store_frames", C.c_int64), ("lang_rows", C.c_int32), ("absolute", C.c_int32)]
 
@@ -113,7 +117,7 @@
            "hulc_k_plan_kl_sample", "hulc_k_st_softmax_bwd", "hulc_k_plan_gather", "hulc_k_plan_scatter_grad", "hulc_k_normal_kl_sample", "hulc_k_normal_rsample_bwd",
            "hulc_k_layernorm_fwd", "hulc_k_layernorm_bwd", "hulc_k_layernorm_mean", "hulc_k_tr_layer_fwd", "hulc_k_tr_ffn_bwd", "hulc_k_tr_attn_bwd",
            "hulc_k_window_compact", "hulc_k_rows_expand", "hulc_k_rows_reduce", "hulc_k_gemm_epi", "hulc_k_gemm_multi", "hulc_k_gemm_pick", "hulc_k_gemm_wgrad_nsplit",
-           "hulc_k_det_head_loss", "hulc_k_det_head_bwd", "hulc_k_det_head_act",
+           "hulc_k_det_head_loss", "hulc_k_det_head_bwd", "hulc_k_det_head_act", "hulc_k_unpack_sweep", "hulc_k_adam_pack",
            "hulc_k_conv_wgrad_t", "hulc_k_conv1_wgrad_u8_t", "hulc_k_conv_tile_t", "hulc_k_conv_pair_t", "hulc_k_conv_plan"]
 
 _lib = None
@@ -274,6 +278,10 @@
         lib.hulc_k_conv_tile_t.argtypes = [I, I, P, P, P, P, P, P, I, I, I, I, I, P]
         lib.hulc_k_conv_pair_t.argtypes = [I, I, C.POINTER(HulcConvJob), C.POINTER(HulcConvJob), I, I, PI, P]
         lib.hulc_k_conv_plan.argtypes = [I, I, I, I, I, PI, PI, PI, PI]
+    if hasattr(lib, "hulc_k_unpack_sweep") or not os.environ.get("HULC_LIB_PATH"):
+        P, I, F, U = C.c_void_p, C.c_int32, C.c_float, C.c_uint64
+        lib.hulc_k_unpack_sweep.argtypes = [P, P, I, I, I, I, I, I, I, I, I, C.POINTER(C.c_void_p), C.POINTER(C.c_int64), I, P]
+        lib.hulc_k_adam_pack.argtypes = [I, P, P, P, P, P, C.c_int64, C.POINTER(HulcAdamPackJob), I, F, F, F, F, C.c_int64, F, I, P]
     _lib = lib
     return lib
 
diff --git a/include/hulc_hip.h b/include/hulc_hip.h
--- a/include/hulc_hip.h
+++ b/include/hulc_hip.h
@@ -272,6 +272,11 @@
                           void* out_t, void* dpp_t, void* hip_stream);
 int hulc_k_plan_gather(int32_t dtype, const void* w_t, const int32_t* idx, int32_t B, int32_t NCAT, int32_t NCLS, int32_t H, const float* b1, const float* b2, float* out,
                        const void* emb, void* embg, int32_t S, int32_t W, const void* goal, int32_t G, int32_t grow0, void* cb, void* hip_stream);
+int hulc_k_unpack_sweep(const float* part, float* grad, int32_t O, int32_t I, int32_t KH, int32_t KW, int32_t nhwc, int32_t nsplit, int32_t ysplit, int32_t yparts, int32_t nzero,
+                        float* const* zp, const int64_t* zn, int32_t zblocks, void* hip_stream);
+typedef struct hulc_adam_pack_job { int64_t base; int32_t n, kind; int32_t a[5]; void* d0; void* d1; float* f0; } hulc_adam_pack_job;
+int hulc_k_adam_pack(int32_t dtype, float* p, const float* g, float* m, float* v, void* shadow, int64_t numel, const hulc_adam_pack_job* jobs, int32_t n_jobs, float lr,
+                     float beta1, float beta2, float eps, int64_t step, float weight_decay, int32_t decoupled, void* hip_stream);
 int hulc_k_plan_scatter_grad(int32_t dtype, int32_t form, const void* dC, const int32_t* idx, int32_t B, int32_t NCAT, int32_t NCLS, int32_t H, int32_t KIN, float* dw,
                              int32_t store, void* hip_stream);
 int hulc_k_normal_kl_sample(int32_t dtype, const float* pr_state, const float* pp_state, int32_t B, int32_t n, const float* eps_in, float* eps_out, float* plan_f, void* plan_t,
```

Result: no change. 21870 windows/s (median of 2 runs) (+0.1%).
